# funkelab/cellulus

Measured on AMD Instinct MI355X. Metric: train crops/sec (U-Net fwd+bwd + OCE loss + Adam), higher is better.
Workload: dtype f32 (exact 3xbf16 operand split, 6 products, f32 accumulate)

## Files before the change

### cellulus_amd/_clx.py

```python

import ctypes
import os
from ctypes import POINTER, Structure, c_char_p, c_double, c_int, c_longlong, c_size_t, c_void_p

import torch

_HERE = os.path.dirname(os.path.abspath(__file__))
LIB_PATH = os.path.join(_HERE, "libclx.so")


class ClxError(RuntimeError):
    """A libclx entry point returned a negative status."""


class ClxSrc(Structure):

    _fields_ = [
        ("ptr", c_void_p),
        ("C", c_int),
        ("ld", c_int),
        ("D", c_int),
        ("H", c_int),
        ("W", c_int),
        ("oz", c_int),
        ("oy", c_int),
        ("ox", c_int),
        ("fz", c_int),
        ("fy", c_int),
        ("fx", c_int),
    ]


class ClxPackJob(Structure):

    _fields_ = [("w", c_void_p), ("wp", c_void_p), ("cout", c_int), ("cin", c_int), ("taps", c_int),
                ("cin_pad", c_int), ("cout_pad", c_int), ("mode", c_int)]


class ClxConvDesc(Structure):

    _fields_ = [
        ("nsrc", c_int),
        ("src", ClxSrc * 2),
        ("B", c_int),
        ("ID", c_int),
        ("IH", c_int),
        ("IW", c_int),
        ("KD", c_int),
        ("KH", c_int),
        ("KW", c_int),
        ("PD", c_int),
        ("PH", c_int),
        ("PW", c_int),
        ("N", c_int),
        ("wpack", c_void_p),
        ("bias", c_void_p),
        ("relu", c_int),
        ("mask", c_void_p),
        ("ld_mask", c_int),
        ("out", c_void_p),
        ("ld_out", c_int),
        ("accumulate", c_int),
        ("algo", c_int),
        ("workspace", c_void_p),
        ("workspace_bytes", c_size_t),
        ("vcache", c_void_p),
        ("vcache_valid", c_int),
        ("c_real", c_int),
        ("dy_vcache", c_void_p),
        ("gate_out", c_void_p),
        ("ld_gate", c_int),
        ("mask_bits", c_void_p),
        ("ld_mask_bits", c_int),
        ("det_turns", c_void_p),
        ("adjoint", c_int),
        ("pool_out", c_void_p),
        ("ld_pool", c_int),
        ("tile_list", c_void_p),
        ("tile_count", c_int),
        ("precision", c_int),
        ("wplanes", c_void_p),
        ("aplanes", c_void_p),
        ("aplanes_valid", c_int),
        ("dyplanes", c_void_p),
        ("dyplanes_valid", c_int),
        ("out_planes", c_void_p),
        ("out_colsum", c_void_p),
    ]


_P = c_void_p
_I = c_int
_LL = c_longlong
_D = c_double

PROTOTYPES = {
    "clx_last_error": (c_char_p, []),
    "clx_abi_version": (_I, []),
    "clx_device_count": (_I, []),
    "clx_profile_enable": (_I, [_I]),
    "clx_profile_read": (_I, [_I, POINTER(c_double), POINTER(c_double), POINTER(c_double)]),
    "clx_profile_clock": (_I, [POINTER(c_double), POINTER(c_double), _I]),
    "clx_conv_fwd": (_I, [POINTER(ClxConvDesc), _P]),
    "clx_conv_wgrad": (_I, [POINTER(ClxConvDesc), _P, _I, _P, _P, _P]),
    "clx_chain64_fwd": (_I, [_P, _I, _LL, _P, _P, _P, _I, _P, _I, _P, _P, _I, _I, _P, _I, _P, _I, _P]),
    "clx_chain64_bwd": (_I, [_P, _I, _I, _P, _I, _P, _I, _I, _LL, _P, _P, _P, _I, _P, _P, _P, _P, _P]),
    "clx_pack_weights": (_I, [_P, _P, _I, _I, _I, _I, _I, _I, _P]),
    "clx_pack_weights_batch": (_I, [_P, _I, _LL, _P]),
    "clx_unpack_wgrad": (_I, [_P, _P, _I, _I, _I, _I, _I, _P]),
    "clx_unpack_wgrad_wino": (_I, [_P, _P, _I, _I, _I, _I, _I, _I, _I, _P]),
    "clx_conv_workspace_bytes": (c_size_t, [POINTER(ClxConvDesc), _I]),
    "clx_conv_vcache_bytes": (c_size_t, [POINTER(ClxConvDesc), _I]),
    "clx_conv_sp_covers": (_I, [POINTER(ClxConvDesc), _I]),
    "clx_planes_bytes": (c_size_t, [_LL, _I]),
    "clx_split_planes": (_I, [_P, _LL, _LL, _I, _P, _P]),
    "clx_join_planes": (_I, [_P, _LL, _I, _P, _LL, _P]),
    "clx_gemm_planes": (_I, [_P, _P, _I, _I, _I, _P, _I, _P, _I, _P]),
    "clx_wgrad_planes": (_I, [_P, _P, _LL, _I, _I, _P, _I, _P]),
    "clx_conv_fused_applicable": (_I, [POINTER(ClxConvDesc)]),
    "clx_conv_fused_workspace_bytes": (c_size_t, [POINTER(ClxConvDesc)]),
    "clx_planar_to_pixel": (_I, [_P, _P, _I, _I, _LL, _I, _P]),
    "clx_pixel_to_planar": (_I, [_P, _P, _I, _I, _LL, _I, _P]),
    "clx_depth_to_space": (_I, [_P, _I, _P, _I, _I, _I, _I, _I, _I, _I, _I, _I, _P]),
    "clx_space_to_depth": (_I, [_P, _I, _P, _I, _I, _I, _I, _I, _I, _I, _I, _I, _P]),
    "clx_subpixel_split_weights": (_I, [_P, _P, _P] + [_I] * 10 + [_P]),
    "clx_subpixel_fold_grads": (_I, [_P, _P, _P] + [_I] * 10 + [_P]),
    "clx_maxpool_fwd": (_I, [_P, _P, _I, _I, _I, _I, _I, _I, _I, _I, _P]),
    "clx_changed_rows_workspace": (c_size_t, [_I, _I, _I, _I]),
    "clx_changed_rows": (_I, [_P, _P, _I, _I, _I, _I, _I, _I, _I, _I, _I, _P, _P, _LL, _P, _P]),
    "clx_changed_tiles": (_I, [_P, _I, _I, _I, _I, _I, _I, _I, _I, _I, _I, _I, _P, _P, _LL, _P]),
    "clx_grey_rows": (_I, [_P, _I, _I, _I, _I, _I, _P, _LL, _P, _P, _I, _I, _P, _I, _P]),
    "clx_conv_first_dgrad": (_I, [_P, _I, _P, _I, _I, _I, _I, _I, _I, _I, _P, _P]),
    "clx_gather_rows": (_I, [_P, _I, _P, _LL, _I, _P, _I, _P]),
    "clx_scatter_rows": (_I, [_P, _I, _P, _LL, _I, _P, _I, _P]),
    "clx_broadcast_rows": (_I, [_P, _LL, _P, _I, _P]),
    "clx_maxpool_bwd": (_I, [_P, _P, _P, _P] + [_I] * 7 + [_P] + [_I] * 8 + [_P]),
    "clx_upsample_bwd": (_I, [_P] + [_I] * 8 + [_P, _P] + [_I] * 8 + [_P]),
    "clx_gather_add_fwd": (_I, [_P, _P, _P, _I, _I, _I, _I, _I, _I, _P, _P]),
    "clx_gather_add_bwd": (_I, [_P, _P, _P, _I, _I, _I, _I, _I, _I, _P, _P]),
    "clx_oce_loss_fwd_bwd": (_I, [_P, _P, _P, _P, _LL, _I, ctypes.c_float, ctypes.c_float, ctypes.c_float, _P]),
    "clx_conv_wgrad_turns_bytes": (c_size_t, [POINTER(ClxConvDesc)]),
    "clx_colsum_scratch_bytes": (c_size_t, [_I]),
    "clx_colsum_ordered": (_I, [_P, _I, _LL, _I, _P, _P, _P]),
    "clx_oce_pairs_det_scratch_bytes": (c_size_t, [_I, _I, _LL]),
    "clx_oce_pairs_fused_det": (_I, [_P, _P, _P, _P, _P, _I, _I, _I, _I, _I, _I, ctypes.c_float, ctypes.c_float, _P, _P]),
    "clx_oce_pairs_fused": (_I, [_P, _P, _P, _P, _P, _I, _I, _I, _I, _I, _I, ctypes.c_float, ctypes.c_float, _P]),
    "clx_sample_pairs": (_I, [_P, _P, _P, _I, _I, _I, _I, _I, _I, POINTER(c_int), ctypes.c_ulonglong,
                              ctypes.c_ulonglong, _P]),
    "clx_adam_step": (_I, [_P, _P, _P, _P, _LL, _D, _D, _D, _D, _D, _I, _P]),
    "clx_adam_step_guarded": (_I, [_P, _P, _P, _P, _LL, _D, _D, _D, _D, _D, _I, _P, _P]),
    "clx_noise_stats": (_I, [_P, _P, _I, _I, _LL, _P]),
    "clx_noise_inject": (_I, [_P, _P, _P, _I, _I, _LL, ctypes.c_float, _P]),
    "clx_zero_many": (_I, [POINTER(_P), POINTER(_LL), _I, _P]),
    "clx_gather_rows_f64": (_I, [_P, _P, _LL, _I, _P, _P]),
    "clx_rows_extent_f64": (_I, [_P, _LL, _I, _P, _P]),
    "clx_noise_stats_minmax": (_I, [_P, _P, _I, _I, _LL, _P, _I, _P]),
    "clx_ms_prepare_workspace": (c_size_t, [_LL]),
    "clx_ms_prepare": (_I, [_P, _P, _D, _I, _I, _I, _I, _P, _P, _P, _P, _P]),
    "clx_ms_prepare_f32": (_I, [_P, _P, _D, _I, _I, _I, _I, _P, _P, _P, _P, _P]),
    "clx_ms_iterate": (_I, [_P, _I, _P, _I, _I, _D, _I, _P, _P, _P, _P]),
    "clx_ms_iterate_grid": (_I, [_P, _I, _P, POINTER(c_double), _D, _I, _I, _I, _P, _I, _I, _D, _I,
                                 _P, _P, _P, _P]),
    "clx_ms_assign": (_I, [_P, _P, _I, _P, _I, _I, _P, _P]),
    "clx_ms_assign_grid": (_I, [_P, _P, _I, _P, _I, _I, _P, _P, POINTER(c_double), _D, _I, _I, _I, _P, _P]),
    "clx_ms_assign_cells": (_I, [_P, _P, _I, _P, _I, _I, _P, _P, POINTER(c_double), _D, _I, _I, _I, _P, _P]),
    "clx_ms_assign_dense": (_I, [_P, _P, _I, _I, _P, _P, POINTER(c_double), _D, _I, _I, _I, _P, _I, _I, _I, _I, _P, _P]),
    "clx_ms_dedup_centers": (_I, [_P, _P, _I, _I, _D, _P, POINTER(_I)]),
    "clx_sample_offsets_mt19937": (_I, [_P, POINTER(_I), _I, _I, _LL, _P, POINTER(_I)]),
    "clx_elastic_crop_workspace": (c_size_t, [_I, POINTER(c_int), _I]),
    "clx_elastic_crop": (_I, [_P, _I, _I, _I, _I, POINTER(c_int), POINTER(c_int), POINTER(c_int), ctypes.c_float, _I, _I,
                              _P, _P, _P, _P, _P, _P]),
    "clx_ms_bucket_workspace": (c_size_t, [_I, _LL]),
    "clx_ms_bucket": (_I, [_P, _I, _I, POINTER(c_double), _D, _I, _I, _I, _P, _P, _P, _P]),
    "clx_offset_magnitude": (_I, [_P, _P, _I, _LL, _P]),
    "clx_gaussian_filter_f64": (_I, [_P, _P, _P, _I, _I, _I, _P, _I, _P]),
    "clx_negate_f64": (_I, [_P, _P, _LL, _P]),
    "clx_peak_local_max": (_I, [_P, _I, _I, _I, _P, _P, _I, _P, _P]),
    "clx_greedy_cluster": (_I, [_P, _P, _I, _I, _I, _D, _I, _D, _I, _P, _P, _P, _P]),
    "clx_cc_workspace": (c_size_t, [_LL]),
    "clx_cc_label_filter": (_I, [_P, _P, _I, _I, _I, _I, _P, _P, _P]),
    "clx_edt_workspace": (c_size_t, [_LL]),
    "clx_edt_sq": (_I, [_P, _P, _I, _I, _I, _I, _P, _P]),
    "clx_grow_shrink": (_I, [_P, _I, _I, _I, _I, _I, _P, _P]),
    "clx_minmax_f64": (_I, [_P, _LL, _P, _P]),
    "clx_histogram_f64": (_I, [_P, _LL, _P, _I, _P, _P]),
    "clx_minmax_f32": (_I, [_P, _LL, _P, _P]),
    "clx_histogram_f32": (_I, [_P, _LL, _P, _I, _P, _P]),
    "clx_inst_stats": (_I, [_P, _P, _I, _I, _I, _I, _I, _P, _P, _P]),
    "clx_inst_histogram": (_I, [_P, _P, _I, _LL, _P, _I, _P, _I, _P, _P]),
    "clx_inst_refine": (_I, [_P, _P, _I, _I, _I, _I, _I, _P, _P, _P, _P, _P, _I, _P, _P]),
    "clx_lz4_decompress": (_LL, [_P, _LL, _P, _LL]),
    "clx_blosclz_decompress": (_LL, [_P, _LL, _P, _LL]),
    "clx_blosc_compress_bound": (_LL, [_LL]),
    "clx_blosc_compress_lz4": (_LL, [_P, _LL, _I, _I, _P, _LL]),
    "clx_unshuffle_bytes": (_I, [_P, _P, _LL, _I]),
    "clx_label_presence": (_I, [_P, _LL, _I, _P, _P, _P]),
# ... 90 lines not shown
```

### cellulus_amd/csrc/clx_common.h

```cpp
#pragma once
#include <hip/hip_runtime.h>
#include <hip/hip_ext.h>
#include <stdint.h>
#include <stdio.h>
#include <stdarg.h>
#include "../../include/clx.h"

void clx_set_error(const char* fmt, ...);

#define CLX_REQUIRE(cond, ...)                \
  do {                                        \
    if (!(cond)) {                            \
      clx_set_error(__VA_ARGS__);             \
      return CLX_ERR_ARG;                     \
    }                                         \
  } while (0)

#define CLX_CHECK_LAUNCH(name)                                           \
  do {                                                                   \
    hipError_t e__ = hipGetLastError();                                  \
    if (e__ != hipSuccess) {                                             \
      clx_set_error("%s: launch failed: %s", name, hipGetErrorString(e__)); \
      return CLX_ERR_LAUNCH;                                             \
    }                                                                    \
  } while (0)

typedef float f32x4 __attribute__((ext_vector_type(4)));
typedef float f32x16 __attribute__((ext_vector_type(16)));

struct FastDiv {
  uint32_t m, l, d;
};
static inline FastDiv make_fastdiv(uint32_t d) {
  FastDiv f;
  f.d = d;
  uint32_t l = 0;
  while ((1ull << l) < d) ++l;
  f.l = l;
  f.m = (uint32_t)(((1ull << 32) * ((1ull << l) - d)) / d + 1);
  return f;
}
__device__ __forceinline__ uint32_t fdiv(uint32_t n, const FastDiv& f) {
  return (__umulhi(f.m, n) + n) >> f.l;
}

__device__ __forceinline__ int xcd_remap(int bid, int nblocks) {
  const int q = nblocks >> 3, r = nblocks & 7;
  const int xcd = bid & 7, idx = bid >> 3;
  const int base = (xcd < r) ? xcd * (q + 1) : r * (q + 1) + (xcd - r) * q;
  return base + idx;
}

static inline int cdiv(long long a, long long b) { return (int)((a + b - 1) / b); }

bool clx_smallc_applicable(const clx_conv_desc* d);
int clx_smallc_fwd(const clx_conv_desc* d, hipStream_t st);
int clx_smallc_wgrad(const clx_conv_desc* d, const float* dy, int ld_dy, float* dwpack,
                     float* dbias, hipStream_t st);

int clx_igemm_launch(const clx_conv_desc* d, int batch, long long bs_in, long long bs_w,
                     long long bs_out, hipStream_t st);
int clx_wgrad_launch(const clx_conv_desc* d, const float* dy, int ld_dy, float* dwpack, float* dbias,
                     int batch, long long bs_x, long long bs_dy, long long bs_out, hipStream_t st);
bool clx_sp_fwd_rule(const clx_conv_desc* d);
bool clx_sp_wgrad_rule(const clx_conv_desc* d);
bool clx_sp_applicable(const clx_conv_desc* d);
bool clx_wino_sp(const clx_conv_desc* d);
int clx_sp_launch(const void* A, const void* B, int M, int N, int K, long long rows_a, int batch, long long bs_a, long long bs_b,
                  long long bs_out, const clx_conv_desc* ep, hipStream_t st);
int clx_sp_clock_read(double* shader_ticks, double* wall_ticks, int reset);
int clx_sp_split(const float* x, long long ld, long long rows, int K, void* planes, float* colsum, int nreal, hipStream_t st);
int clx_sp_wgrad_launch(const void* dy_planes, const void* x_planes, long long rows, int N, int C, int batch, long long bs_dy,
                        long long bs_x, long long bs_out, float* dw, int ld_dw, hipStream_t st);
int clx_wino_fwd(const clx_conv_desc* d, hipStream_t st);
int clx_wino_wgrad(const clx_conv_desc* d, const float* dy, int ld_dy, float* dwpack, float* dbias,
                   hipStream_t st);
int clx_wino_pack(const float* w, float* wp, int cout, int cin, int cin_pad, int cout_pad, int dgrad, int tile,
                  int ksize, int kd, hipStream_t st);

int clx_wino_fused_fwd(const clx_conv_desc* d, hipStream_t st);

bool clx_prof_enabled();
void clx_prof_events(int kind, double flops, hipEvent_t* e0, hipEvent_t* e1);
#define CLX_LAUNCH_TIMED(kernel, grid, block, st, e0, e1, ...) \
  hipExtLaunchKernelGGL(kernel, grid, block, 0, st, e0, e1, 0, __VA_ARGS__)
#define CLX_LAUNCH_KIND(kind, kernel, grid, block, lds, st, ...)                              \
  do {                                                                                        \
    hipEvent_t e0__ = nullptr, e1__ = nullptr;                                                \
    if (clx_prof_enabled()) clx_prof_events(kind, 0.0, &e0__, &e1__);                         \
    hipExtLaunchKernelGGL(kernel, grid, block, lds, st, e0__, e1__, 0, __VA_ARGS__);          \
  } while (0)
```

### cellulus_amd/csrc/conv_igemm.hip

```cpp
#include "clx_common.h"
#include <stdlib.h>

__device__ unsigned long long g_clk_ticks[2];
extern "C" int clx_profile_clock(double* shader_ticks, double* wall_ticks_100mhz, int reset) {
  unsigned long long h[2] = {0ull, 0ull};
  if (hipMemcpyFromSymbol(h, HIP_SYMBOL(g_clk_ticks), sizeof(h)) != hipSuccess) {
    clx_set_error("clx_profile_clock: copy failed");
    return CLX_ERR_LAUNCH;
  }
  double sc = 0.0, sw = 0.0;
  if (clx_sp_clock_read(&sc, &sw, reset) != CLX_OK) {
    clx_set_error("clx_profile_clock: copy failed");
    return CLX_ERR_LAUNCH;
  }
  if (shader_ticks) *shader_ticks = (double)h[0] + sc;
  if (wall_ticks_100mhz) *wall_ticks_100mhz = (double)h[1] + sw;
  if (reset) {
    const unsigned long long z[2] = {0ull, 0ull};
    if (hipMemcpyToSymbol(HIP_SYMBOL(g_clk_ticks), z, sizeof(z)) != hipSuccess) {
      clx_set_error("clx_profile_clock: reset failed");
      return CLX_ERR_LAUNCH;
    }
  }
  return CLX_OK;
// ... 400 lines not shown
    } else if (n_live) {
#pragma unroll 1
      for (int j = 0; j < PH; ++j) {
        if (!live[j]) continue;
        float* dst = out_base + (size_t)mrow[j] * p.ld_out;
        for (int e = 0; e < 4 && n + e < p.N; ++e) {
          float x = val[j][e];
          if (p.mask) x = (p.mask[(size_t)mrow[j] * p.ld_mask + n + e] > 0.f) ? x : 0.f;
          dst[e] = x;
        }
      }
    }
  }
  if (clk_block) { atomicAdd(&g_clk_ticks[0], clock64() - clk_c0); atomicAdd(&g_clk_ticks[1], wall_clock64() - clk_w0); }
}

}

static const float* zero_buffer() {
  static const float* cache[64] = {nullptr};
  int dev = 0;
  if (hipGetDevice(&dev) != hipSuccess || dev < 0 || dev >= 64) return nullptr;
  if (cache[dev] == nullptr) {
    void* ptr = nullptr;
    if (hipGetSymbolAddress(&ptr, HIP_SYMBOL(g_zero16)) != hipSuccess) return nullptr;
    cache[dev] = (const float*)ptr;
  }
  return cache[dev];
}

static int conv_validate(const clx_conv_desc* d, const char* who) {
  CLX_REQUIRE(d != nullptr, "%s: null descriptor", who);
  CLX_REQUIRE(d->nsrc == 1 || d->nsrc == 2, "%s: nsrc must be 1 or 2", who);
  CLX_REQUIRE(d->B > 0 && d->ID > 0 && d->IH > 0 && d->IW > 0, "%s: bad extent", who);
  const int K[3] = {d->KD, d->KH, d->KW};
  const int P[3] = {d->PD, d->PH, d->PW};
  const int I[3] = {d->ID, d->IH, d->IW};
  for (int i = 0; i < 3; ++i) {
    CLX_REQUIRE(K[i] >= 1 && K[i] <= 3, "%s: kernel extent must be 1, 2 or 3", who);
    CLX_REQUIRE(P[i] >= 0 && P[i] < K[i], "%s: padding must be < kernel extent", who);
    CLX_REQUIRE(I[i] + 2 * P[i] - K[i] + 1 > 0, "%s: input smaller than kernel", who);
  }
  for (int s = 0; s < d->nsrc; ++s) {
    const clx_src& S = d->src[s];
    CLX_REQUIRE(S.ptr != nullptr, "%s: null source %d", who, s);
    CLX_REQUIRE(S.C > 0 && S.C % 4 == 0 && S.ld % 4 == 0 && S.ld >= S.C,
                "%s: source channels/ld must be multiples of 4 (C=%d ld=%d)", who, S.C, S.ld);
    CLX_REQUIRE(((uintptr_t)S.ptr & 15) == 0, "%s: source pointer must be 16-byte aligned", who);
    CLX_REQUIRE(S.fz >= 1 && S.fy >= 1 && S.fx >= 1, "%s: upsample factors >= 1", who);
    CLX_REQUIRE(S.oz >= 0 && S.oy >= 0 && S.ox >= 0, "%s: negative crop", who);
    CLX_REQUIRE((d->ID - 1 + S.oz) / S.fz < S.D && (d->IH - 1 + S.oy) / S.fy < S.H &&
                    (d->IW - 1 + S.ox) / S.fx < S.W,
                "%s: source %d smaller than the logical input", who, s);
  }
  const long long M = (long long)d->B * (d->ID + 2 * d->PD - d->KD + 1) *
                      (d->IH + 2 * d->PH - d->KH + 1) * (d->IW + 2 * d->PW - d->KW + 1);
  CLX_REQUIRE(M < (1ll << 31), "%s: too many output pixels", who);
  return CLX_OK;
}

static void fill_params(const clx_conv_desc* d, ConvP& p) {
  p.nsrc = d->nsrc;
  for (int s = 0; s < 2; ++s) {
    const clx_src& S = d->src[s < d->nsrc ? s : 0];
    p.src[s] = SrcP{S.ptr, S.C, S.ld, S.D, S.H, S.W, S.oz, S.oy, S.ox, S.fz, S.fy, S.fx};
  }
  p.B = d->B; p.ID = d->ID; p.IH = d->IH; p.IW = d->IW;
  p.KD = d->KD; p.KH = d->KH; p.KW = d->KW;
  p.PD = d->PD; p.PH = d->PH; p.PW = d->PW;
  p.OD = d->ID + 2 * d->PD - d->KD + 1;
  p.OH = d->IH + 2 * d->PH - d->KH + 1;
  p.OW = d->IW + 2 * d->PW - d->KW + 1;
  p.N = d->N;
  p.M = d->B * p.OD * p.OH * p.OW;
  p.Ctot = d->src[0].C + (d->nsrc == 2 ? d->src[1].C : 0);
  p.Ktot = p.Ctot * d->KD * d->KH * d->KW;
  p.dOW = make_fastdiv(p.OW); p.dOH = make_fastdiv(p.OH); p.dOD = make_fastdiv(p.OD);
  p.wpack = d->wpack; p.bias = d->bias; p.mask = d->mask; p.out = d->out;
  p.gate_out = d->gate_out; p.ld_gate = d->ld_gate; p.mask_bits = d->mask_bits; p.ld_mask_bits = d->ld_mask_bits;
  p.relu = d->relu; p.ld_mask = d->ld_mask; p.ld_out = d->ld_out;
  p.accumulate = d->accumulate;
  p.bs_in = p.bs_w = p.bs_out = 0;
  p.flush_every = 0;
}

extern "C" int clx_conv_fwd(const clx_conv_desc* d, clx_stream stream) {
  int rc = conv_validate(d, "clx_conv_fwd");
  if (rc) return rc;
  CLX_REQUIRE(d->wpack && d->out, "clx_conv_fwd: null wpack/out");
  CLX_REQUIRE(d->N > 0 && d->ld_out >= d->N, "clx_conv_fwd: bad N/ld_out");
  CLX_REQUIRE(((uintptr_t)d->wpack & 15) == 0, "clx_conv_fwd: wpack must be 16-byte aligned");
  CLX_REQUIRE(d->mask == nullptr || (d->ld_mask >= d->N && d->ld_mask % 4 == 0 &&
                                     ((uintptr_t)d->mask & 15) == 0),
              "clx_conv_fwd: mask must be 16-byte aligned with ld_mask %% 4 == 0 and >= N");
  CLX_REQUIRE(d->ld_out % 4 == 0 && ((uintptr_t)d->out & 15) == 0,
              "clx_conv_fwd: out must be 16-byte aligned with ld_out %% 4 == 0");
  CLX_REQUIRE(d->gate_out == nullptr || (d->relu && d->ld_out % 32 == 0 && d->ld_gate * 32 >= d->ld_out),
              "clx_conv_fwd: gate_out needs relu, ld_out %% 32 == 0 and ld_gate >= ld_out / 32");
  CLX_REQUIRE(d->mask_bits == nullptr || (d->mask == nullptr && d->ld_mask_bits * 32 >= d->N),
              "clx_conv_fwd: mask_bits replaces mask and needs ld_mask_bits >= ceil(N / 32)");
  CLX_REQUIRE(d->algo == CLX_ALGO_DIRECT || d->algo == CLX_ALGO_WINOGRAD || d->algo == CLX_ALGO_WINOGRAD4 ||
                  d->algo == CLX_ALGO_WINOGRAD4_FUSED,
              "clx_conv_fwd: bad algo");
  CLX_REQUIRE((d->out_planes == nullptr && d->out_colsum == nullptr && !d->aplanes_valid) ||
                  (d->algo == CLX_ALGO_DIRECT && d->aplanes != nullptr && clx_sp_applicable(d)),
              "clx_conv_fwd: out_planes / out_colsum / aplanes_valid need the split-precision 1x1 product "
              "(clx_conv_sp_covers, wplanes and aplanes)");
  if (d->algo == CLX_ALGO_WINOGRAD4_FUSED) return clx_wino_fused_fwd(d, (hipStream_t)stream);
  if (d->algo != CLX_ALGO_DIRECT) return clx_wino_fwd(d, (hipStream_t)stream);
  CLX_REQUIRE(d->pool_out == nullptr && d->tile_list == nullptr && !d->adjoint,
              "clx_conv_fwd: pool_out / tile_list / adjoint need a Winograd algorithm (algo = %d)", d->algo);
  if (clx_smallc_applicable(d) && d->mask == nullptr && d->mask_bits == nullptr && d->gate_out == nullptr) {
    clx_smallc_fwd(d, (hipStream_t)stream);
    CLX_CHECK_LAUNCH("clx_conv_fwd(small-channel)");
    return CLX_OK;
  }
  rc = clx_igemm_launch(d, 1, 0, 0, 0, (hipStream_t)stream);
  if (rc) return rc;
  CLX_CHECK_LAUNCH("clx_conv_fwd");
  return CLX_OK;
}

int clx_igemm_launch(const clx_conv_desc* d, int batch, long long bs_in, long long bs_w,
                     long long bs_out, hipStream_t st) {
  if (batch == 1 && d->aplanes != nullptr && clx_sp_applicable(d)) {
    const clx_src& S = d->src[0];
    const long long M = (long long)d->B * d->ID * d->IH * d->IW;
    if (!d->aplanes_valid) {
      const int rc = clx_sp_split(S.ptr, S.ld, M, S.C, d->aplanes, nullptr, 0, st);
      if (rc) return rc;
    }
    return clx_sp_launch(d->aplanes, d->wplanes, (int)M, d->N, S.C, M, 1, 0, 0, 0, d, st);
  }
  ConvP p;
  fill_params(d, p);
  p.zeros = zero_buffer();
  CLX_REQUIRE(p.zeros != nullptr, "clx_conv_fwd: cannot resolve the device zero buffer");
  p.bs_in = bs_in; p.bs_w = bs_w; p.bs_out = bs_out;
  static const int flush_env = getenv("CLX_IGEMM_FLUSH") ? atoi(getenv("CLX_IGEMM_FLUSH")) : 2;
  p.flush_every = flush_env > 0 ? flush_env : 0;
  const bool wide = d->N > 64 && (double)(cdiv(d->N, 128) * 128) / d->N <= 1.2;
  hipEvent_t e0 = nullptr, e1 = nullptr;
  if (clx_prof_enabled())
    clx_prof_events(wide ? CLX_PROF_IGEMM_WIDE : CLX_PROF_IGEMM_NARROW, 2.0 * p.M * p.N * p.Ktot * batch, &e0, &e1);
  static const bool fast_env = getenv("CLX_IGEMM_FAST") == nullptr || atoi(getenv("CLX_IGEMM_FAST")) != 0;
  int fast = fast_env && (long long)p.N * p.Ktot < (1ll << 30) ? 1 : 0;
  const bool padded = d->PD != 0 || d->PH != 0 || d->PW != 0;
  for (int s = 0; s < d->nsrc && fast; ++s) {
    const clx_src& S = d->src[s];
    const long long floats = (long long)d->B * S.D * S.H * S.W * S.ld;
    if (S.C % BK != 0 || floats >= (padded ? (1ll << 29) : (1ll << 30))) fast = 0;
  }
  if (fast && padded) fast = 2;
  static const bool dbg = getenv("CLX_IGEMM_DEBUG") != nullptr;
  if (dbg) fprintf(stderr, "igemm fast=%d wide=%d M=%d N=%d K=%d batch=%d pad=%d%d%d k=%d%d%d nsrc=%d C0=%d\n", (int)fast, (int)wide, p.M, p.N, p.Ktot, batch, d->PD, d->PH, d->PW, d->KD, d->KH, d->KW, d->nsrc, d->src[0].C);
  if (wide) {
    p.nbm = cdiv(p.M, 128); p.nbn = cdiv(p.N, 128);
    if (fast == 1) CLX_LAUNCH_TIMED((conv_igemm_kernel<128, 128, 2, 2, 1>), dim3(p.nbm * p.nbn, batch), dim3(256), st, e0, e1, p);
    else if (fast == 2) CLX_LAUNCH_TIMED((conv_igemm_kernel<128, 128, 2, 2, 2>), dim3(p.nbm * p.nbn, batch), dim3(256), st, e0, e1, p);
    else CLX_LAUNCH_TIMED((conv_igemm_kernel<128, 128, 2, 2>), dim3(p.nbm * p.nbn, batch), dim3(256), st, e0, e1, p);
  } else {
    p.nbm = cdiv(p.M, 128); p.nbn = cdiv(p.N, 64);
    if (fast == 1) CLX_LAUNCH_TIMED((conv_igemm_kernel<128, 64, 4, 1, 1>), dim3(p.nbm * p.nbn, batch), dim3(256), st, e0, e1, p);
    else if (fast == 2) CLX_LAUNCH_TIMED((conv_igemm_kernel<128, 64, 4, 1, 2>), dim3(p.nbm * p.nbn, batch), dim3(256), st, e0, e1, p);
    else CLX_LAUNCH_TIMED((conv_igemm_kernel<128, 64, 4, 1>), dim3(p.nbm * p.nbn, batch), dim3(256), st, e0, e1, p);
  }
  return CLX_OK;
}
```

### cellulus_amd/csrc/conv_smallc.hip

```cpp
#include "clx_common.h"

namespace {

struct SmallP {
  const float* x;
  int ld_x, B, D, H, W;
  int oz, oy, ox;
  int ID, IH, IW, KD, KH, KW, PD, PH, PW, OD, OH, OW;
  int N, M, taps;
  FastDiv dOW, dOH, dOD;
  const float* wpack;
  const float* bias;
  float* out;
  int ld_out, relu;
  const float* dy;
  int ld_dy;
  float* dwp;
  float* dbias;
  int tiles_per_block;
  int RX, items;
  FastDiv dRX;
};

constexpr int PT = 64;
constexpr int MAX_TAPS = 27;

template <int PTILE>
__device__ __forceinline__ void stage_patch(const SmallP& p, int m0, float* Xs) {
  static_assert(256 % PTILE == 0, "a thread keeps one pixel of the tile");
  const int K4 = p.taps;
  const int pl = threadIdx.x % PTILE;
  const uint32_t m = (uint32_t)(m0 + pl);
  const bool live = m < (uint32_t)p.M;
  const uint32_t q1 = fdiv(m, p.dOW);
  const int ox = (int)(m - q1 * p.OW);
  const uint32_t q2 = fdiv(q1, p.dOH);
  const int oy = (int)(q1 - q2 * p.OH);
  const uint32_t q3 = fdiv(q2, p.dOD);
  const int oz = (int)(q2 - q3 * p.OD);
  const int b = (int)q3;
  int tx = 0, ty = 0, tz = 0;
  {
    const int tap = threadIdx.x / PTILE;
    tx = tap % p.KW; ty = (tap / p.KW) % p.KH; tz = tap / (p.KW * p.KH);
  }
  constexpr int STEP = 256 / PTILE;
  for (int tap = threadIdx.x / PTILE; tap < K4; tap += STEP) {
    f32x4 v = {0.f, 0.f, 0.f, 0.f};
    const int lz = oz + tz - p.PD, ly = oy + ty - p.PH, lx = ox + tx - p.PW;
    if (live && (unsigned)lz < (unsigned)p.ID && (unsigned)ly < (unsigned)p.IH && (unsigned)lx < (unsigned)p.IW) {
      const long long pix = (((long long)b * p.D + lz + p.oz) * p.H + ly + p.oy) * p.W + lx + p.ox;
      v = *reinterpret_cast<const f32x4*>(p.x + pix * p.ld_x);
    }
    *reinterpret_cast<f32x4*>(&Xs[(pl * K4 + tap) * 4]) = v;
    tx += STEP;
    while (tx >= p.KW) { tx -= p.KW; if (++ty == p.KH) { ty = 0; ++tz; } }
  }
}

template <int NG>
__global__ __launch_bounds__(256) void conv_smallc_fwd_kernel(const SmallP p) {
  constexpr int PL = 256 / NG;
  constexpr int PPT = PT / PL;
  extern __shared__ float smem[];
  const int K = p.taps * 4;
  float* Ws = smem;
  float* Xs = smem + K * NG * 4;
  const int n0 = blockIdx.y * NG * 4;
  const int ng = threadIdx.x % NG, pl = threadIdx.x / NG;
  __shared__ int used_channels;
  if (threadIdx.x == 0) used_channels = 0;
  __syncthreads();
  int mine_used = 0;
  for (int idx = threadIdx.x; idx < K * NG * 4; idx += 256) {
    const int n = idx / K, k = idx % K;
    const float wv = (n0 + n < p.N) ? p.wpack[(size_t)(n0 + n) * K + k] : 0.f;
    Ws[k * NG * 4 + n] = wv;
    if (wv != 0.f) mine_used |= 1 << (k & 3);
  }
  if (mine_used) atomicOr(&used_channels, mine_used);
  const int n = n0 + ng * 4;
  f32x4 bv = {0.f, 0.f, 0.f, 0.f};
  if (p.bias && n < p.N) {
#pragma unroll
    for (int e = 0; e < 4; ++e) bv[e] = (n + e < p.N) ? p.bias[n + e] : 0.f;
  }
  for (int t = 0; t < p.tiles_per_block; ++t) {
    const int m0 = (blockIdx.x * p.tiles_per_block + t) * PT;
    if (m0 >= p.M) break;
    __syncthreads();
    stage_patch<PT>(p, m0, Xs);
    __syncthreads();
    f32x4 acc[PPT];
#pragma unroll
    for (int i = 0; i < PPT; ++i) acc[i] = bv;
    const int used = used_channels;
    for (int c = 0; c < 4; ++c) {
// ... 47 lines not shown
  const long long per = (long long)p.tiles_per_block;
  const long long m_begin = (long long)blockIdx.x * per;
  const long long m_end = m_begin + per < p.M ? m_begin + per : p.M;
  const bool live = n < p.N;
  const int gtap = tap0 + (g < ntap ? g : 0);
  const int my_tx = gtap % p.KW - p.PW, my_ty = (gtap / p.KW) % p.KH - p.PH, my_tz = gtap / (p.KW * p.KH) - p.PD;
  for (long long mm = m_begin + q; mm < m_end; mm += Q) {
    const uint32_t m = (uint32_t)mm;
    const uint32_t q1 = fdiv(m, p.dOW);
    const int ox = (int)(m - q1 * p.OW);
    const uint32_t q2 = fdiv(q1, p.dOH);
    const int oy = (int)(q1 - q2 * p.OH);
    const uint32_t q3 = fdiv(q2, p.dOD);
    const int oz = (int)(q2 - q3 * p.OD);
    const int b = (int)q3;
    f32x4 dyv = {0.f, 0.f, 0.f, 0.f};
    if (live) dyv = *reinterpret_cast<const f32x4*>(p.dy + (size_t)m * p.ld_dy + n);
    if (tap0 == 0) bsum += dyv;
    if constexpr (G >= 16) {
      f32x4 mine = {0.f, 0.f, 0.f, 0.f};
      if (g < ntap) {
        const int lz = oz + my_tz, ly = oy + my_ty, lx = ox + my_tx;
        if ((unsigned)lz < (unsigned)p.ID && (unsigned)ly < (unsigned)p.IH && (unsigned)lx < (unsigned)p.IW) {
          const long long pix = (((long long)b * p.D + lz + p.oz) * p.H + ly + p.oy) * p.W + lx + p.ox;
          mine = *reinterpret_cast<const f32x4*>(p.x + pix * p.ld_x);
        }
      }
#pragma unroll
      for (int a = 0; a < MT; ++a) {
        if (a < ntap) {
          f32x4 xv;
#pragma unroll
          for (int c = 0; c < 4; ++c) {
            xv[c] = __shfl(mine[c], (int)(threadIdx.x & 63 & ~(G - 1)) + a, 64);
          }
#pragma unroll
          for (int c = 0; c < 4; ++c) acc[a][c] += xv[c] * dyv;
        }
      }
    } else {
#pragma unroll
      for (int a = 0; a < MT; ++a) {
        if (a < ntap) {
          const int tap = tap0 + a;
          const int lz = oz + tap / (p.KW * p.KH) - p.PD, ly = oy + (tap / p.KW) % p.KH - p.PH, lx = ox + tap % p.KW - p.PW;
          f32x4 xv = {0.f, 0.f, 0.f, 0.f};
          if ((unsigned)lz < (unsigned)p.ID && (unsigned)ly < (unsigned)p.IH && (unsigned)lx < (unsigned)p.IW) {
            const long long pix = (((long long)b * p.D + lz + p.oz) * p.H + ly + p.oy) * p.W + lx + p.ox;
            xv = *reinterpret_cast<const f32x4*>(p.x + pix * p.ld_x);
          }
#pragma unroll
          for (int c = 0; c < 4; ++c) acc[a][c] += xv[c] * dyv;
        }
      }
    }
  }
  __syncthreads();
#pragma unroll
  for (int a = 0; a < MT; ++a) {
    if (a < ntap) {
#pragma unroll
      for (int c = 0; c < 4; ++c)
#pragma unroll
        for (int e = 0; e < 4; ++e) atomicAdd(&red[(a * 4 + c) * NT + g * 4 + e], acc[a][c][e]);
    }
  }
#pragma unroll
  for (int e = 0; e < 4; ++e) atomicAdd(&red[ntap * 4 * NT + g * 4 + e], bsum[e]);
  __syncthreads();
  for (int i = threadIdx.x; i < ntap * 4 * NT; i += 256) {
    const int nl = i % NT, c = (i / NT) & 3, tap = tap0 + i / (4 * NT);
    if (n0 + nl < p.N) atomicAdd(p.dwp + ((size_t)tap * p.N + n0 + nl) * 4 + c, red[i]);
  }
  if (p.dbias && tap0 == 0)
    for (int i = threadIdx.x; i < NT; i += 256)
      if (n0 + i < p.N) atomicAdd(p.dbias + n0 + i, red[ntap * 4 * NT + i]);
}

struct Run {
  int ox0, m0;
  long long base;
};

__device__ __forceinline__ Run decode_run(const SmallP& p, uint32_t item) {
  const uint32_t q1 = fdiv(item, p.dRX);
  const int rx = (int)(item - q1 * p.RX);
  const uint32_t q2 = fdiv(q1, p.dOH);
  const int oy = (int)(q1 - q2 * p.OH);
  const uint32_t q3 = fdiv(q2, p.dOD);
  const int oz = (int)(q2 - q3 * p.OD);
  const int b = (int)q3;
  Run r;
  r.ox0 = rx * 4;
  r.m0 = ((b * p.OD + oz) * p.OH + oy) * p.OW + r.ox0;
  r.base = (((long long)b * p.D + oz + p.oz) * p.H + oy + p.oy) * p.W + r.ox0 + p.ox;
  return r;
}

template <int KD>
struct GreyLane {
  static constexpr int R = KD * 3, NP = R * 6, TAPS = R * 3;
  int px, cq, col;
  long long poff;
  __device__ __forceinline__ GreyLane(const SmallP& p) {
    const int lane = threadIdx.x & 63;
    px = lane >> 4; cq = lane & 15;
    const int l = lane < NP ? lane : 0;
    const int r = l / 6;
    col = l - r * 6;
    const int tz = r / 3, ty = r - tz * 3;
    poff = ((long long)tz * p.H + ty) * p.W;
  }
  __device__ __forceinline__ float load_patch(const SmallP& p, const Run& r) const {
    const int c = r.ox0 + col < p.IW ? col : p.IW - 1 - r.ox0;
    return p.x[(r.base + poff + c) * p.ld_x];
  }
  __device__ __forceinline__ float tap(float pv, int row, int tx) const {
    return __shfl(pv, row * 6 + tx + px, 64);
  }
};

template <int KD>
__global__ __launch_bounds__(256) void conv_grey_fwd_kernel(const SmallP p) {
  using L = GreyLane<KD>;
  const L ln(p);
  const int wave = __builtin_amdgcn_readfirstlane(threadIdx.x >> 6);
  const int n = blockIdx.y * 64 + ln.cq * 4;
  const bool live_n = n < p.N;
  f32x4 w[L::TAPS];
#pragma unroll
  for (int t = 0; t < L::TAPS; ++t)
#pragma unroll
    for (int e = 0; e < 4; ++e) w[t][e] = live_n ? p.wpack[((size_t)(n + e) * L::TAPS + t) * 4] : 0.f;
  f32x4 bv = {0.f, 0.f, 0.f, 0.f};
  if (p.bias && live_n) bv = *reinterpret_cast<const f32x4*>(p.bias + n);
  const uint32_t last = (uint32_t)p.items - 1, stride = gridDim.x * 4;
  uint32_t item = blockIdx.x * 4 + wave;
  Run r[3];
  float pv[3];
#pragma unroll
  for (int s = 0; s < 2; ++s) {
    r[s] = decode_run(p, item + s * stride < last ? item + s * stride : last);
    pv[s] = ln.load_patch(p, r[s]);
  }
  while (true) {
#pragma unroll
    for (int s = 0; s < 3; ++s) {
      if (item > last) return;
      const int s2 = (s + 2) % 3;
      const uint32_t nxt = item + 2 * stride;
      r[s2] = decode_run(p, nxt < last ? nxt : last);
      pv[s2] = ln.load_patch(p, r[s2]);
      f32x4 acc = bv;
#pragma unroll
      for (int row = 0; row < L::R; ++row)
#pragma unroll
        for (int tx = 0; tx < 3; ++tx) acc += ln.tap(pv[s], row, tx) * w[row * 3 + tx];
      if (p.relu) {
#pragma unroll
        for (int e = 0; e < 4; ++e) acc[e] = fmaxf(acc[e], 0.f);
      }
      if (live_n && r[s].ox0 + ln.px < p.OW)
        *reinterpret_cast<f32x4*>(p.out + (size_t)(r[s].m0 + ln.px) * p.ld_out + n) = acc;
      item += stride;
    }
  }
}

template <int KD>
__global__ __launch_bounds__(256) void conv_grey_wgrad_kernel(const SmallP p) {
  using L = GreyLane<KD>;
  __shared__ float red[(L::TAPS + 1) * 64];
  const L ln(p);
  const int wave = __builtin_amdgcn_readfirstlane(threadIdx.x >> 6);
  const int n0 = blockIdx.y * 64, n = n0 + ln.cq * 4;
  const bool live_n = n < p.N;
  const int nld = live_n ? n : 0;
  for (int i = threadIdx.x; i < (L::TAPS + 1) * 64; i += 256) red[i] = 0.f;
  f32x4 acc[L::TAPS];
#pragma unroll
  for (int t = 0; t < L::TAPS; ++t) acc[t] = f32x4{0.f, 0.f, 0.f, 0.f};
  f32x4 bsum = {0.f, 0.f, 0.f, 0.f};
  const uint32_t last = (uint32_t)p.items - 1, stride = gridDim.x * 4;
  uint32_t item = blockIdx.x * 4 + wave;
  auto load_dy = [&](const Run& r) {
    const int m = r.ox0 + ln.px < p.OW ? r.m0 + ln.px : r.m0;
    return *reinterpret_cast<const f32x4*>(p.dy + (size_t)m * p.ld_dy + nld);
  };
  Run r[3];
  float pv[3];
  f32x4 dy[3];
#pragma unroll
  for (int s = 0; s < 2; ++s) {
    r[s] = decode_run(p, item + s * stride < last ? item + s * stride : last);
    pv[s] = ln.load_patch(p, r[s]);
    dy[s] = load_dy(r[s]);
  }
  bool more = item <= last;
  while (more) {
#pragma unroll
    for (int s = 0; s < 3; ++s) {
      if (more) {
        const int s2 = (s + 2) % 3;
        const uint32_t nxt = item + 2 * stride;
        r[s2] = decode_run(p, nxt < last ? nxt : last);
        pv[s2] = ln.load_patch(p, r[s2]);
        dy[s2] = load_dy(r[s2]);
        const bool ok = live_n && r[s].ox0 + ln.px < p.OW;
        f32x4 dyv;
#pragma unroll
        for (int e = 0; e < 4; ++e) dyv[e] = ok ? dy[s][e] : 0.f;
        bsum += dyv;
#pragma unroll
        for (int row = 0; row < L::R; ++row)
#pragma unroll
          for (int tx = 0; tx < 3; ++tx) acc[row * 3 + tx] += ln.tap(pv[s], row, tx) * dyv;
        item += stride;
        more = item <= last;
      }
    }
  }
  __syncthreads();
#pragma unroll
  for (int t = 0; t < L::TAPS; ++t)
#pragma unroll
    for (int e = 0; e < 4; ++e) atomicAdd(&red[t * 64 + ln.cq * 4 + e], acc[t][e]);
#pragma unroll
  for (int e = 0; e < 4; ++e) atomicAdd(&red[L::TAPS * 64 + ln.cq * 4 + e], bsum[e]);
  __syncthreads();
  for (int i = threadIdx.x; i < L::TAPS * 64; i += 256) {
    const int nl = i & 63, t = i >> 6;
    if (n0 + nl < p.N) atomicAdd(p.dwp + ((size_t)t * p.N + n0 + nl) * 4, red[i]);
  }
  if (p.dbias && threadIdx.x < 64 && n0 + threadIdx.x < p.N)
    atomicAdd(p.dbias + n0 + threadIdx.x, red[L::TAPS * 64 + threadIdx.x]);
}

template <int KD>
__global__ __launch_bounds__(256) void conv_grey_rows_kernel(const float* __restrict__ x, int D, int H, int W, int OD,
                                                             int OH, int OW, const int* __restrict__ rows, long long n,
                                                             const float* __restrict__ wpack,
                                                             const float* __restrict__ bias, int relu, int N,
                                                             float* __restrict__ out, int ld_out) {
  constexpr int R = KD * 3, TAPS = R * 3;
  const int lane = threadIdx.x & 63, px = lane >> 4, cq = lane & 15;
  const int nn = blockIdx.y * 64 + cq * 4;
  const bool live_n = nn < N;
  f32x4 w[TAPS];
#pragma unroll
  for (int t = 0; t < TAPS; ++t)
#pragma unroll
    for (int e = 0; e < 4; ++e) w[t][e] = live_n ? wpack[((size_t)(nn + e) * TAPS + t) * 4] : 0.f;
  f32x4 bv = {0.f, 0.f, 0.f, 0.f};
  if (bias && live_n) bv = *reinterpret_cast<const f32x4*>(bias + nn);
  const long long npo = (long long)OD * OH * OW;
  const long long groups = (n + 3) / 4;
  for (long long g = (long long)blockIdx.x * 4 + (threadIdx.x >> 6); g < groups; g += (long long)gridDim.x * 4) {
    const long long r = g * 4 + px;
    const bool live = r < n;
    const long long row = rows[live ? r : n - 1];
    const long long b = row / npo, pix = row - b * npo;
    const int ox = (int)(pix % OW), oy = (int)((pix / OW) % OH), oz = (int)(pix / ((long long)OW * OH));
    const float* src = x + ((b * D + oz) * H + oy) * (long long)W + ox;
    float xv[TAPS];
#pragma unroll
    for (int rr = 0; rr < R; ++rr)
#pragma unroll
      for (int tx = 0; tx < 3; ++tx) xv[rr * 3 + tx] = src[((long long)(rr / 3) * H + (rr % 3)) * W + tx];
    f32x4 acc = bv;
#pragma unroll
    for (int rr = 0; rr < R; ++rr)
#pragma unroll
      for (int tx = 0; tx < 3; ++tx) acc += xv[rr * 3 + tx] * w[rr * 3 + tx];
    if (relu) {
#pragma unroll
      for (int e = 0; e < 4; ++e) acc[e] = fmaxf(acc[e], 0.f);
    }
    if (live && live_n) *reinterpret_cast<f32x4*>(out + (size_t)r * ld_out + nn) = acc;
  }
}

bool grey_applicable(const clx_conv_desc* d, int ld_act) {
  return d->c_real == 1 && d->KH == 3 && d->KW == 3 && (d->KD == 1 || d->KD == 3) && d->PD == 0 &&
         d->PH == 0 && d->PW == 0 && d->N % 4 == 0 && ld_act % 4 == 0;
}

dim3 grey_grid(SmallP& p) {
  p.RX = cdiv(p.OW, 4);
  p.items = p.B * p.OD * p.OH * p.RX;
  p.dRX = make_fastdiv(p.RX);
  const int ny = cdiv(p.N, 64);
  int nx = 768 / ny;
  if (nx < 1) nx = 1;
  if (nx > cdiv(p.items, 4)) nx = cdiv(p.items, 4);
  return dim3(nx, ny);
}

bool fill(const clx_conv_desc* d, SmallP& p) {
  const clx_src& S = d->src[0];
  p.x = S.ptr; p.ld_x = S.ld; p.B = d->B; p.D = S.D; p.H = S.H; p.W = S.W;
  p.oz = S.oz; p.oy = S.oy; p.ox = S.ox;
  p.ID = d->ID; p.IH = d->IH; p.IW = d->IW;
  p.KD = d->KD; p.KH = d->KH; p.KW = d->KW;
  p.PD = d->PD; p.PH = d->PH; p.PW = d->PW;
  p.OD = d->ID + 2 * d->PD - d->KD + 1;
  p.OH = d->IH + 2 * d->PH - d->KH + 1;
  p.OW = d->IW + 2 * d->PW - d->KW + 1;
  p.N = d->N;
  p.M = d->B * p.OD * p.OH * p.OW;
  p.taps = d->KD * d->KH * d->KW;
  p.dOW = make_fastdiv(p.OW); p.dOH = make_fastdiv(p.OH); p.dOD = make_fastdiv(p.OD);
  return true;
}

int pick_ng(int N) {
  int ng = 4;
  while (ng < 64 && ng * 4 < N) ng *= 2;
  return ng;
}

}

bool clx_smallc_applicable(const clx_conv_desc* d) {
  if (d->nsrc != 1 || d->accumulate) return false;
  const clx_src& S = d->src[0];
  if (S.C != 4 || S.fz != 1 || S.fy != 1 || S.fx != 1) return false;
  const int taps = d->KD * d->KH * d->KW;
  return taps > 1 && taps <= MAX_TAPS && d->N >= 4;
}

int clx_smallc_fwd(const clx_conv_desc* d, hipStream_t st) {
  SmallP p{};
  fill(d, p);
  p.wpack = d->wpack; p.bias = d->bias; p.out = d->out; p.ld_out = d->ld_out; p.relu = d->relu;
  if (grey_applicable(d, d->ld_out) && ((uintptr_t)d->out & 15) == 0 && (!d->bias || ((uintptr_t)d->bias & 15) == 0)) {
    const dim3 grid = grey_grid(p);
    if (d->KD == 1) conv_grey_fwd_kernel<1><<<grid, 256, 0, st>>>(p);
    else conv_grey_fwd_kernel<3><<<grid, 256, 0, st>>>(p);
    return CLX_OK;
  }
  const int ng = pick_ng(p.N);
  const int K = p.taps * 4;
  const int tiles = cdiv(p.M, PT);
  p.tiles_per_block = tiles > 4096 ? 4 : 1;
  const dim3 grid(cdiv(tiles, p.tiles_per_block), cdiv(p.N, ng * 4));
  const size_t lds = (size_t)(K * ng * 4 + PT * K) * sizeof(float);
  switch (ng) {
    case 4: conv_smallc_fwd_kernel<4><<<grid, 256, lds, st>>>(p); break;
    case 8: conv_smallc_fwd_kernel<8><<<grid, 256, lds, st>>>(p); break;
    case 16: conv_smallc_fwd_kernel<16><<<grid, 256, lds, st>>>(p); break;
    case 32: conv_smallc_fwd_kernel<32><<<grid, 256, lds, st>>>(p); break;
    default: conv_smallc_fwd_kernel<64><<<grid, 256, lds, st>>>(p); break;
  }
  return CLX_OK;
}

int clx_smallc_wgrad(const clx_conv_desc* d, const float* dy, int ld_dy, float* dwpack,
                     float* dbias, hipStream_t st) {
  SmallP p{};
  fill(d, p);
  p.dy = dy; p.ld_dy = ld_dy; p.dwp = dwpack; p.dbias = dbias;
  if (grey_applicable(d, ld_dy) && ((uintptr_t)dy & 15) == 0) {
    const dim3 grid = grey_grid(p);
    if (d->KD == 1) conv_grey_wgrad_kernel<1><<<grid, 256, 0, st>>>(p);
    else conv_grey_wgrad_kernel<3><<<grid, 256, 0, st>>>(p);
    return CLX_OK;
  }
  const int ng = pick_ng(p.N);
  const int blocks = p.M < 512 * 64 ? cdiv(p.M, 64) : 512;
  p.tiles_per_block = cdiv(p.M, blocks);
  const dim3 grid(cdiv(p.M, p.tiles_per_block), cdiv(p.N, ng * 4), cdiv(p.taps, 9));
  const size_t lds = (size_t)((p.taps < 9 ? p.taps : 9) * 4 * ng * 4 + ng * 4) * sizeof(float);
  switch (ng) {
    case 4: conv_smallc_wgrad_stream_kernel<4><<<grid, 256, lds, st>>>(p); break;
    case 8: conv_smallc_wgrad_stream_kernel<8><<<grid, 256, lds, st>>>(p); break;
    case 16: conv_smallc_wgrad_stream_kernel<16><<<grid, 256, lds, st>>>(p); break;
    case 32: conv_smallc_wgrad_stream_kernel<32><<<grid, 256, lds, st>>>(p); break;
    default: conv_smallc_wgrad_stream_kernel<64><<<grid, 256, lds, st>>>(p); break;
  }
  return CLX_OK;
}

extern "C" int clx_grey_rows(const float* x, int B, int ID, int IH, int IW, int KD, const int* rows, long long n,
                             const float* wpack, const float* bias, int relu, int N, float* out, int ld_out,
                             clx_stream stream) {
  CLX_REQUIRE(n >= 0, "clx_grey_rows: bad count");
  if (n == 0) return CLX_OK;
  CLX_REQUIRE(x && rows && wpack && out, "clx_grey_rows: null pointer");
  CLX_REQUIRE(B > 0 && (KD == 1 || KD == 3) && ID >= KD && IH >= 3 && IW >= 3, "clx_grey_rows: a 3x3 or 3x3x3 window");
  CLX_REQUIRE(N > 0 && N % 4 == 0 && ld_out % 4 == 0 && ld_out >= N && ((uintptr_t)out & 15) == 0 &&
                  (!bias || ((uintptr_t)bias & 15) == 0),
              "clx_grey_rows: N, ld_out multiples of 4, aligned out / bias");
  const int OD = ID - KD + 1, OH = IH - 2, OW = IW - 2;
  long long gx = (n + 15) / 16;
  if (gx > 4096) gx = 4096;
  const dim3 grid((unsigned)gx, (unsigned)((N + 63) / 64));
  hipStream_t st = (hipStream_t)stream;
  if (KD == 1) conv_grey_rows_kernel<1><<<grid, 256, 0, st>>>(x, ID, IH, IW, OD, OH, OW, rows, n, wpack, bias, relu, N, out, ld_out);
  else conv_grey_rows_kernel<3><<<grid, 256, 0, st>>>(x, ID, IH, IW, OD, OH, OW, rows, n, wpack, bias, relu, N, out, ld_out);
  CLX_CHECK_LAUNCH("clx_grey_rows");
  return CLX_OK;
}
```

### cellulus_amd/csrc/gemm_sp.hip

```cpp
#include "clx_common.h"
#include "sp_planes.h"
#include <stdlib.h>
#include <type_traits>

__device__ unsigned long long g_sp_clk_ticks[2];
int clx_sp_clock_read(double* shader_ticks, double* wall_ticks, int reset) {
  unsigned long long h[2] = {0ull, 0ull};
  if (hipMemcpyFromSymbol(h, HIP_SYMBOL(g_sp_clk_ticks), sizeof(h)) != hipSuccess) return CLX_ERR_LAUNCH;
  *shader_ticks = (double)h[0];
  *wall_ticks = (double)h[1];
  if (reset) {
    const unsigned long long z[2] = {0ull, 0ull};
    if (hipMemcpyToSymbol(HIP_SYMBOL(g_sp_clk_ticks), z, sizeof(z)) != hipSuccess) return CLX_ERR_LAUNCH;
  }
  return CLX_OK;
}

namespace {

typedef __bf16 bf16x8 __attribute__((ext_vector_type(8)));
using sp::u32x2;
using sp::u32x4;
using sp::FRAG;
using sp::KSTEP;
// ... 31 lines not shown
    if constexpr (COLSUM) { s0 += v0; s1 += v1; }
    u32x2 a0, a1, a2, b0, b1, b2;
    split4(v0, a0, a1, a2);
    split4(v1, b0, b1, b2);
    char* dst = out + f * KSTEP + lane * 16;
    *reinterpret_cast<u32x4*>(dst) = u32x4{a0[0], a0[1], b0[0], b0[1]};
    *reinterpret_cast<u32x4*>(dst + FRAG) = u32x4{a1[0], a1[1], b1[0], b1[1]};
    *reinterpret_cast<u32x4*>(dst + 2 * FRAG) = u32x4{a2[0], a2[1], b2[0], b2[1]};
  }
  if constexpr (COLSUM) {
    if (w0 < nfrag) {
      const int ks = (int)(w0 % ksteps);
#pragma unroll
      for (int e = 0; e < 4; ++e) {
#pragma unroll
        for (int m = 1; m < 32; m <<= 1) { s0[e] += __shfl_xor(s0[e], m, 64); s1[e] += __shfl_xor(s1[e], m, 64); }
      }
      if (r == 0) {
#pragma unroll
        for (int e = 0; e < 4; ++e) {
          const int k0 = ks * 16 + h * 8 + e;
          if (k0 < nreal) atomicAdd(colsum + k0, s0[e]);
          if (k0 + 4 < nreal) atomicAdd(colsum + k0 + 4, s1[e]);
        }
      }
    }
  }
}

__global__ __launch_bounds__(256) void sp_join_kernel(const char* __restrict__ in, long long ld, long long rows, int ksteps,
                                                      float* __restrict__ x, long long nfrag) {
  const int lane = threadIdx.x & 63;
  const long long w0 = ((long long)blockIdx.x * blockDim.x + threadIdx.x) >> 6, nw = ((long long)gridDim.x * blockDim.x) >> 6;
  const int r = lane & 31, h = lane >> 5;
  for (long long f = w0; f < nfrag; f += nw) {
    const int ks = (int)(f % ksteps);
    const long long rb = f / ksteps;
    const long long row = rb * 32 + r;
    if (row >= rows) continue;
    const char* src = in + f * KSTEP + lane * 16;
    const u32x4 q0 = *reinterpret_cast<const u32x4*>(src), q1 = *reinterpret_cast<const u32x4*>(src + FRAG),
                q2 = *reinterpret_cast<const u32x4*>(src + 2 * FRAG);
    float* dst = x + row * ld + ks * 16 + h * 8;
#pragma unroll
    for (int e = 0; e < 8; ++e) {
      const int sh = (e & 1) * 16;
      const float f0 = __uint_as_float(((q0[e >> 1] >> sh) & 0xffffu) << 16);
      const float f1 = __uint_as_float(((q1[e >> 1] >> sh) & 0xffffu) << 16);
      const float f2 = __uint_as_float(((q2[e >> 1] >> sh) & 0xffffu) << 16);
      dst[e] = (f0 + f1) + f2;
    }
  }
}

__global__ __launch_bounds__(256) void sp_zero_tail_kernel(char* __restrict__ planes, long long bs, long long rows, int ksteps) {
  const long long rb0 = rows >> 5, rb1 = sp::padded_rows(rows) / 32;
  const int per_rb = ksteps * 6 * 32;
  const long long total = (rb1 - rb0) * per_rb;
  for (long long i = (long long)blockIdx.x * blockDim.x + threadIdx.x; i < total; i += (long long)gridDim.x * blockDim.x) {
    const long long rb = rb0 + i / per_rb;
    const int k = (int)(i % per_rb), r = k & 31, q = k >> 5;
    if (rb * 32 + r >= rows)
      *reinterpret_cast<u32x4*>(planes + blockIdx.y * bs + rb * ksteps * (long long)KSTEP + (long long)q * 512 + r * 16) = u32x4{0u, 0u, 0u, 0u};
  }
}

struct SpP {
  const char* A;
  const char* B;
  long long bs_a, bs_b, bs_out;
  float* out;
  int M, N, ksteps;
  int rb_a;
  int rb_b;
  const float* bias;
  const float* mask;
  const unsigned int* mask_bits;
  unsigned int* gate_out;
  const float* zeros;
  int relu, accumulate, ld_out, ld_mask, ld_mask_bits, ld_gate;
  int nbm, nbn;
  char* out_planes;
  float* colsum; int colsum_n;
  unsigned int stride_a, stride_b;
  int total_steps, steps_per_slice, nslices;
};

template <int BM = SP_BM, int NWAVES = 8, int BN = SP_BN>
__device__ __forceinline__ void sp_epilogue_from_lds(const SpP& p, const float* Cs, int m0, int n0, int batch, int tid, int lane) {
  constexpr int WPR = BN / 32;
  constexpr int LDC = BN + 4;
  constexpr int PASS_ROWS = NWAVES / WPR * 8;
  constexpr int ITERS = BM / PASS_ROWS;
  constexpr int PH = 8;
  static_assert(ITERS % PH == 0, "whole groups of passes");
  const int wv = tid >> 6;
  const int c4 = (wv % WPR) * 32 + (lane & 7) * 4;
  const int row0 = (wv / WPR) * 8 + (lane >> 3);
  const int n = n0 + c4;
  const bool n_live = n < p.N;
  f32x4 csum = {0.f, 0.f, 0.f, 0.f};
  const long long prow = p.out_planes ? sp::padded_rows(p.M) : 0;
#pragma unroll 1
  for (int h0 = 0; h0 < ITERS; h0 += PH) {
    f32x4 val[PH];
    int mrow[PH];
    bool live[PH];
#pragma unroll
    for (int j = 0; j < PH; ++j) {
      const int row = row0 + PASS_ROWS * (h0 + j);
      mrow[j] = m0 + row;
      live[j] = mrow[j] < p.M && n_live;
      val[j] = *reinterpret_cast<const f32x4*>(&Cs[row * LDC + c4]);
    }
    float* const out_base = p.out + batch * p.bs_out + n;
    if (p.accumulate) {
      f32x4 prev[PH];
#pragma unroll
      for (int j = 0; j < PH; ++j)
        prev[j] = *reinterpret_cast<const f32x4*>(live[j] ? out_base + (size_t)mrow[j] * p.ld_out : p.zeros);
#pragma unroll
      for (int j = 0; j < PH; ++j) val[j] += prev[j];
    }
    if (p.relu) {
#pragma unroll
      for (int j = 0; j < PH; ++j)
#pragma unroll
        for (int e = 0; e < 4; ++e) val[j][e] = fmaxf(val[j][e], 0.f);
    }
    if (p.mask_bits) {
      unsigned int wd[PH];
#pragma unroll
      for (int j = 0; j < PH; ++j) wd[j] = live[j] ? p.mask_bits[(size_t)mrow[j] * p.ld_mask_bits + (n >> 5)] : 0u;
#pragma unroll
      for (int j = 0; j < PH; ++j)
#pragma unroll
        for (int e = 0; e < 4; ++e) val[j][e] = ((wd[j] >> ((n & 31) + e)) & 1u) ? val[j][e] : 0.f;
    }
    if (p.gate_out) {
#pragma unroll
      for (int j = 0; j < PH; ++j) {
        unsigned int nib = 0u;
#pragma unroll
        for (int e = 0; e < 4; ++e) nib |= (live[j] && val[j][e] > 0.f) ? (1u << e) : 0u;
        unsigned int word = nib << (4 * (lane & 7));
        word |= __shfl_xor(word, 1, 64);
        word |= __shfl_xor(word, 2, 64);
        word |= __shfl_xor(word, 4, 64);
        if ((lane & 7) == 0 && mrow[j] < p.M && n_live) p.gate_out[(size_t)mrow[j] * p.ld_gate + (n >> 5)] = word;
      }
    }
    if (p.mask) {
      f32x4 mk[PH];
#pragma unroll
      for (int j = 0; j < PH; ++j)
        mk[j] = *reinterpret_cast<const f32x4*>(live[j] ? p.mask + (size_t)mrow[j] * p.ld_mask + n : p.zeros);
#pragma unroll
      for (int j = 0; j < PH; ++j)
#pragma unroll
        for (int e = 0; e < 4; ++e) val[j][e] = (!live[j] || mk[j][e] > 0.f) ? val[j][e] : 0.f;
    }
#pragma unroll
    for (int j = 0; j < PH; ++j)
      if (live[j]) *reinterpret_cast<f32x4*>(out_base + (size_t)mrow[j] * p.ld_out) = val[j];
    if (p.out_planes) {
#pragma unroll
      for (int j = 0; j < PH; ++j)
        if (n_live && mrow[j] < prow)
          sp::store4(p.out_planes, mrow[j], n, p.N >> 4, live[j] ? val[j] : f32x4{0.f, 0.f, 0.f, 0.f});
    }
    if (p.colsum) {
#pragma unroll
      for (int j = 0; j < PH; ++j)
        if (live[j]) csum += val[j];
    }
  }
  if (p.colsum) {
#pragma unroll
    for (int e = 0; e < 4; ++e) {
      csum[e] += __shfl_xor(csum[e], 8, 64);
      csum[e] += __shfl_xor(csum[e], 16, 64);
      csum[e] += __shfl_xor(csum[e], 32, 64);
    }
    if ((lane >> 3) == 0 && n_live) {
#pragma unroll
      for (int e = 0; e < 4; ++e)
        if (n + e < p.colsum_n) atomicAdd(p.colsum + n + e, csum[e]);
    }
  }
}

template <int MODE>
__global__ __launch_bounds__(512, 1) void gemm_sp_kernel(const SpP p) {
  __shared__ __attribute__((aligned(16))) char smem[RING * STAGE];
  const int tid = threadIdx.x, lane = tid & 63;
  const int w = __builtin_amdgcn_readfirstlane(tid >> 6);
  const int wm = w >> 1, wn = w & 1;
  int tile_m, tile_n, batch, step0 = 0, ksteps;
  if constexpr (MODE == 0) {
    const int v = xcd_remap(blockIdx.x, p.nbm * p.nbn);
    tile_n = v % p.nbn; tile_m = v / p.nbn;
    batch = blockIdx.y;
    ksteps = p.ksteps;
  } else {
    const int T = p.nbm * p.nbn;
    const int u = xcd_remap(blockIdx.x, gridDim.x);
    const int per_batch = T * p.nslices;
    batch = u / per_batch;
    const int v = u % per_batch;
    const int slice = v / T, t = v % T;
    tile_n = t % p.nbn; tile_m = t / p.nbn;
    step0 = slice * p.steps_per_slice;
    ksteps = p.total_steps - step0 < p.steps_per_slice ? p.total_steps - step0 : p.steps_per_slice;
  }
  const int m0 = tile_m * SP_BM, n0 = tile_n * SP_BN;
  const bool clk_block = blockIdx.x == gridDim.x / 2 && blockIdx.y == gridDim.y / 2 && threadIdx.x == 0;
  unsigned long long clk_c0 = 0, clk_w0 = 0;
  if (clk_block) { clk_c0 = clock64(); clk_w0 = wall_clock64(); }

  const char* const Ab = p.A + batch * p.bs_a;
  const char* const Bb = p.B + batch * p.bs_b;
  auto frag_base = [&](int f) __attribute__((always_inline)) -> const char* {
    if constexpr (MODE == 0) {
      if (f < A_FRAGS) {
        int rb = tile_m * (SP_BM / 32) + f / 3;
        if (rb > p.rb_a - 1) rb = p.rb_a - 1;
        return Ab + ((long long)rb * ksteps * 3 + f % 3) * FRAG;
      }
      const int g = f - A_FRAGS;
      int nb = tile_n * (SP_BN / 32) + g / 3;
      if (nb > p.rb_b - 1) nb = p.rb_b - 1;
      return Bb + ((long long)nb * ksteps * 3 + g % 3) * FRAG;
    } else {
      if (f < A_FRAGS) {
        int cb = tile_m * (SP_BM / 32) + f / 3;
        if (cb > p.M / 32 - 1) cb = p.M / 32 - 1;
        return Ab + ((long long)(2 * cb) * 3 + f % 3) * FRAG;
      }
      const int g = f - A_FRAGS;
      int cb = tile_n * (SP_BN / 32) + g / 3;
      if (cb > p.N / 32 - 1) cb = p.N / 32 - 1;
      return Bb + ((long long)(2 * cb) * 3 + g % 3) * FRAG;
    }
  };
  const char* gsrc[5];
#pragma unroll
  for (int q = 0; q < 4; ++q) gsrc[q] = frag_base(w + 8 * q);
// ... 704 lines not shown
  long long blocks = (nfrag + 3) / 4;
  if (blocks > 8192) blocks = 8192;
  if (colsum != nullptr) {
    if (blocks > 2048) blocks = 2048;
    int g = ksteps % 4 == 0 ? 4 : ksteps % 2 == 0 ? 2 : 1;
    const long long unit = ksteps / g;
    blocks = (blocks + unit - 1) / unit * unit;
    CLX_LAUNCH_KIND(CLX_PROF_SPLIT_PLANES, sp_split_kernel<true>, dim3((unsigned)blocks), dim3(256), 0, st, x, ld, rows, ksteps, (char*)planes,
                    nfrag, colsum, nreal);
  } else {
    CLX_LAUNCH_KIND(CLX_PROF_SPLIT_PLANES, sp_split_kernel<false>, dim3((unsigned)blocks), dim3(256), 0, st, x, ld, rows, ksteps, (char*)planes,
                    nfrag, (float*)nullptr, 0);
  }
  return CLX_OK;
}

extern "C" int clx_split_planes(const float* x, long long ld, long long rows, int K, void* planes, clx_stream stream) {
  const int rc = clx_sp_split(x, ld, rows, K, planes, nullptr, 0, (hipStream_t)stream);
  if (rc) return rc;
  CLX_CHECK_LAUNCH("clx_split_planes");
  return CLX_OK;
}

extern "C" int clx_join_planes(const void* planes, long long rows, int K, float* x, long long ld, clx_stream stream) {
  CLX_REQUIRE(x != nullptr && planes != nullptr, "clx_join_planes: null pointer");
  CLX_REQUIRE(rows > 0 && K > 0 && K % 16 == 0 && ld >= K, "clx_join_planes: K must be a multiple of 16, ld >= K");
  const long long nfrag = sp::padded_rows(rows) / 32 * (K / 16);
  long long blocks = (nfrag + 3) / 4;
  if (blocks > 8192) blocks = 8192;
  sp_join_kernel<<<dim3((unsigned)blocks), dim3(256), 0, (hipStream_t)stream>>>((const char*)planes, ld, rows, K / 16, x, nfrag);
  CLX_CHECK_LAUNCH("clx_join_planes");
  return CLX_OK;
}

static bool sp_pointwise(const clx_conv_desc* d) {
  if ((d->precision != CLX_PREC_F32X3BF16 && d->precision != CLX_PREC_F32X3BF16_G64) || d->nsrc != 1) return false;
  if (d->KD != 1 || d->KH != 1 || d->KW != 1 || d->PD || d->PH || d->PW) return false;
  const clx_src& S = d->src[0];
  if (S.fz != 1 || S.fy != 1 || S.fx != 1 || S.oz || S.oy || S.ox) return false;
  return S.D == d->ID && S.H == d->IH && S.W == d->IW;
}

bool clx_sp_fwd_rule(const clx_conv_desc* d) {
  if (!sp_pointwise(d)) return false;
  const bool g64 = d->precision == CLX_PREC_F32X3BF16_G64;
  return d->N % (g64 ? 64 : SP_BN) == 0 && d->N >= 128 && d->src[0].C % 64 == 0 && d->src[0].C >= 128 && d->ld_out % 4 == 0;
}

bool clx_sp_wgrad_rule(const clx_conv_desc* d) {
  if (!sp_pointwise(d)) return false;
  const int granule = d->precision == CLX_PREC_F32X3BF16_G64 ? 64 : 128;
  if (d->N % granule != 0 || d->src[0].C % granule != 0 || d->N < 128 || d->src[0].C < 128) return false;
  const long long ch = d->N > d->src[0].C ? d->N : d->src[0].C;
  return (long long)d->B * d->ID * d->IH * d->IW * ch * 6 < (1ll << 32) - (1 << 24);
}

bool clx_sp_applicable(const clx_conv_desc* d) { return d->wplanes != nullptr && clx_sp_fwd_rule(d); }

extern "C" int clx_conv_sp_covers(const clx_conv_desc* d, int pass) {
  if (d == nullptr || (pass != CLX_PASS_FWD && pass != CLX_PASS_WGRAD)) return 0;
  if (d->algo == CLX_ALGO_WINOGRAD || d->algo == CLX_ALGO_WINOGRAD4) return clx_wino_sp(d) ? 1 : 0;
  if (d->algo != CLX_ALGO_DIRECT) return 0;
  return (pass == CLX_PASS_FWD ? clx_sp_fwd_rule(d) : clx_sp_wgrad_rule(d)) ? 1 : 0;
}

int clx_sp_launch(const void* A, const void* B, int M, int N, int K, long long rows_a, int batch, long long bs_a, long long bs_b,
                  long long bs_out, const clx_conv_desc* ep, hipStream_t st) {
  CLX_REQUIRE(M > 0 && N > 0 && N % 64 == 0 && K >= 128 && K % 64 == 0,
              "clx_gemm_planes: needs N %% 64 == 0 (whole 128-wide tiles: N %% 128 == 0), K %% 64 == 0 and K >= 128");
  CLX_REQUIRE(rows_a >= M, "clx_gemm_planes: the A planes hold fewer rows than M");
  SpP p = {};
  p.A = (const char*)A; p.B = (const char*)B;
  p.bs_a = bs_a; p.bs_b = bs_b; p.bs_out = bs_out;
  p.out = ep->out; p.ld_out = ep->ld_out;
  p.M = M; p.N = N; p.ksteps = K / 16;
  p.rb_a = (int)(sp::padded_rows(rows_a) / 32);
  p.rb_b = (int)(sp::padded_rows(N) / 32);
  p.bias = ep->bias; p.mask = ep->mask; p.mask_bits = ep->mask_bits; p.gate_out = ep->gate_out;
  p.relu = ep->relu; p.accumulate = ep->accumulate; p.ld_mask = ep->ld_mask; p.ld_mask_bits = ep->ld_mask_bits; p.ld_gate = ep->ld_gate;
  p.zeros = sp_zero_buffer();
  CLX_REQUIRE(p.zeros != nullptr, "clx_gemm_planes: cannot resolve the device zero buffer");
  p.out_planes = batch == 1 ? (char*)ep->out_planes : nullptr;
  p.colsum = batch == 1 ? ep->out_colsum : nullptr; p.colsum_n = N;
  CLX_REQUIRE(p.out_planes == nullptr || ep->ld_out == N, "clx_gemm_planes: out_planes needs a dense output (ld_out == N)");
  p.nbm = cdiv(M, SP_BM); p.nbn = cdiv(N, SP_BN);
  const char* const tile_env = getenv("CLX_SP_TILE");
  const int tile_choice = tile_env != nullptr ? atoi(tile_env) : 0;
  const char* const maxk_env = getenv("CLX_SP_TILE_MAXK");
  const int maxk = maxk_env != nullptr ? atoi(maxk_env) : 1024;
  const bool small_tiles = tile_choice == 128 || (tile_choice != 256 && K <= maxk);
  const char* const shape_env = getenv("CLX_SP_MFMA");
  const bool mfma16 = shape_env != nullptr && atoi(shape_env) == 16 && N % SP_BN == 0;
  hipEvent_t e0 = nullptr, e1 = nullptr;
  if (clx_prof_enabled())
    clx_prof_events(small_tiles && !mfma16 ? CLX_PROF_GEMM_SP2 : CLX_PROF_GEMM_SP, 2.0 * M * N * K * batch, &e0, &e1);
  if (mfma16) CLX_LAUNCH_TIMED(gemm_sp16_kernel, dim3(p.nbm * p.nbn, batch), dim3(512), st, e0, e1, p);
  else if (small_tiles && N % 128 == 0) CLX_LAUNCH_TIMED(gemm_sp2_kernel<128>, dim3(cdiv(M, S2_BM) * (N / 128), batch), dim3(256), st, e0, e1, p);
  else if (small_tiles) CLX_LAUNCH_TIMED(gemm_sp2_kernel<64>, dim3(cdiv(M, S2_BM) * (N / 64), batch), dim3(256), st, e0, e1, p);
  else CLX_LAUNCH_TIMED(gemm_sp_kernel<0>, dim3(p.nbm * p.nbn, batch), dim3(512), st, e0, e1, p);
  return CLX_OK;
}

int clx_sp_wgrad_launch(const void* dy_planes, const void* x_planes, long long rows, int N, int C, int batch, long long bs_dy,
                        long long bs_x, long long bs_out, float* dw, int ld_dw, hipStream_t st) {
  CLX_REQUIRE(rows > 0 && N > 0 && C >= 128 && N % 64 == 0 && C % 64 == 0,
              "clx_wgrad_planes: needs N %% 64 == 0, C %% 64 == 0 and C >= 128");
  SpP p = {};
  p.A = (const char*)dy_planes; p.B = (const char*)x_planes;
  p.bs_a = bs_dy; p.bs_b = bs_x; p.bs_out = bs_out;
  p.out = dw; p.ld_out = ld_dw;
  p.M = N; p.N = C;
  p.stride_a = (unsigned int)(N / 16) * KSTEP; p.stride_b = (unsigned int)(C / 16) * KSTEP;
  CLX_REQUIRE(sp::planes_bytes(rows, N) < (1ll << 32) && sp::planes_bytes(rows, C) < (1ll << 32), "clx_wgrad_planes: operand planes beyond 4 GB");
  p.total_steps = (int)(sp::padded_rows(rows) / 16);
  p.nbm = cdiv(N, SP_BM); p.nbn = cdiv(C, SP_BN);
  const int tiles = p.nbm * p.nbn * batch;
  int cus = 256, dev = 0;
  if (hipGetDevice(&dev) == hipSuccess) (void)hipDeviceGetAttribute(&cus, hipDeviceAttributeMultiprocessorCount, dev);
  int best_ns = 1;
  double best = 1e30;
  const int max_ns = p.total_steps / 8 > 0 ? p.total_steps / 8 : 1;
  for (int ns = 1; ns <= max_ns && ns <= 4096; ++ns) {
    const int sps = (cdiv(p.total_steps, ns) + 7) / 8 * 8;
    const int real_ns = cdiv(p.total_steps, sps);
    if (p.total_steps - (real_ns - 1) * sps < 8) continue;
    const double cost = (double)cdiv((long long)tiles * real_ns, cus) * (sps + 12);
    if (cost < best) { best = cost; best_ns = ns; }
    if ((long long)tiles * ns > 16ll * cus) break;
  }
  p.steps_per_slice = (cdiv(p.total_steps, best_ns) + 7) / 8 * 8;
  p.nslices = cdiv(p.total_steps, p.steps_per_slice);
  CLX_REQUIRE(p.total_steps >= 8 && p.total_steps - (p.nslices - 1) * p.steps_per_slice >= 8, "clx_wgrad_planes: internal: a slice of fewer than 8 steps");
  hipEvent_t e0 = nullptr, e1 = nullptr;
  if (clx_prof_enabled()) clx_prof_events(CLX_PROF_WGRAD_SP, 2.0 * rows * N * C * batch, &e0, &e1);
  CLX_LAUNCH_TIMED(gemm_sp_kernel<1>, dim3(p.nbm * p.nbn * p.nslices * batch), dim3(512), st, e0, e1, p);
  return CLX_OK;
}

extern "C" int clx_wgrad_planes(const void* dy_planes, const void* x_planes, long long rows, int N, int C, float* dw, int ld_dw,
                                clx_stream stream) {
  CLX_REQUIRE(dy_planes && x_planes && dw && ld_dw >= C, "clx_wgrad_planes: null pointer / ld_dw < C");
  const int rc = clx_sp_wgrad_launch(dy_planes, x_planes, rows, N, C, 1, 0, 0, 0, dw, ld_dw, (hipStream_t)stream);
  if (rc) return rc;
  CLX_CHECK_LAUNCH("clx_wgrad_planes");
  return CLX_OK;
}

extern "C" int clx_gemm_planes(const void* a_planes, const void* b_planes, int M, int N, int K, const float* bias, int relu,
                               float* out, int ld_out, clx_stream stream) {
  CLX_REQUIRE(a_planes && b_planes && out, "clx_gemm_planes: null pointer");
  CLX_REQUIRE(ld_out >= N && ld_out % 4 == 0 && ((uintptr_t)out & 15) == 0, "clx_gemm_planes: out must be 16-byte aligned, ld_out %% 4 == 0");
  clx_conv_desc ep = {};
  ep.out = out; ep.ld_out = ld_out; ep.bias = bias; ep.relu = relu;
  const int rc = clx_sp_launch(a_planes, b_planes, M, N, K, M, 1, 0, 0, 0, &ep, (hipStream_t)stream);
  if (rc) return rc;
  CLX_CHECK_LAUNCH("clx_gemm_planes");
  return CLX_OK;
}
```

### cellulus_amd/csrc/wino.hip

```cpp
#include "clx_common.h"
#include "sp_planes.h"
#include "wino_tables.h"

namespace {

inline int grid_for(long long total, int block) {
  long long g = (total + block - 1) / block;
  if (g > 16384) g = 16384;
  if (g < 1) g = 1;
  return (int)g;
}

__device__ __forceinline__ f32x4 ld4(const float* p) { return *reinterpret_cast<const f32x4*>(p); }
__device__ __forceinline__ void st4(float* p, f32x4 v) { *reinterpret_cast<f32x4*>(p) = v; }

struct Geom {
  int B, SH, SW, oy, ox;
  int ID, SD, oz;
  int IH, IW, P;
  int OH, OW, th, tw;
  long long T;
};

template <int MT, int R, bool PL = false>
__global__ __launch_bounds__(256) void wino_input_kernel(const float* __restrict__ x, int ld_x, int C4, Geom g,
                                                         float* __restrict__ V, long long total,
                                                         const int* __restrict__ tile_list = nullptr, long long Tc = 0,
                                                         long long plane_bytes = 0) {
  using W = WT<MT, R>;
  constexpr int A = W::A;
  const int C = C4 * 4;
  const long long Trows = tile_list ? Tc : g.T;
  const long long plane = Trows * C;
  for (long long i = (long long)blockIdx.x * blockDim.x + threadIdx.x; i < total;
       i += (long long)gridDim.x * blockDim.x) {
    int c;
    long long t;
    if constexpr (PL) {
      sp::item_to_row_channel(i, C, t, c);
      if (t >= Trows) continue;
    } else {
      c = (int)(i % C4) * 4;
      t = i / C4;
    }
    const long long tg = tile_list ? (long long)tile_list[t] : t;
    const int tx = (int)(tg % g.tw);
    const long long q = tg / g.tw;
    const int ty = (int)(q % g.th);
    const int b = (int)(q / g.th);
    const int bb = b / g.ID, bz = b - bb * g.ID;
    f32x4 d[A][A];
#pragma unroll
    for (int r = 0; r < A; ++r) {
      const int ly = MT * ty - g.P + r;
#pragma unroll
      for (int s = 0; s < A; ++s) {
        const int lx = MT * tx - g.P + s;
        f32x4 v = {0.f, 0.f, 0.f, 0.f};
        if ((unsigned)ly < (unsigned)g.IH && (unsigned)lx < (unsigned)g.IW) {
          const long long pix = (((long long)bb * g.SD + bz + g.oz) * g.SH + ly + g.oy) * g.SW + lx + g.ox;
          v = ld4(x + pix * ld_x + c);
        }
        d[r][s] = v;
      }
    }
    f32x4 w[A][A];
#pragma unroll
    for (int s = 0; s < A; ++s)
#pragma unroll
      for (int r = 0; r < A; ++r) {
        f32x4 acc = {0.f, 0.f, 0.f, 0.f};
        bool first = true;
#pragma unroll
        for (int k = 0; k < A; ++k) axpy(acc, first, W::BT[r][k], d[k][s]);
        w[r][s] = acc;
      }
    float* dst = V + t * C + c;
#pragma unroll
    for (int r = 0; r < A; ++r)
#pragma unroll
      for (int qq = 0; qq < A; ++qq) {
        f32x4 acc = {0.f, 0.f, 0.f, 0.f};
        bool first = true;
#pragma unroll
        for (int k = 0; k < A; ++k) axpy(acc, first, W::BT[qq][k], w[r][k]);
        if constexpr (PL) sp::store4(reinterpret_cast<char*>(V) + (r * A + qq) * plane_bytes, t, c, C >> 4, acc);
        else st4(dst + (r * A + qq) * plane, acc);
      }
  }
}

template <int MT, int R>
__global__ __launch_bounds__(256) void wino_output_kernel(const float* __restrict__ M, int N4, Geom g,
                                                          const float* __restrict__ bias, int relu,
                                                          const float* __restrict__ mask, int ld_mask,
                                                          float* __restrict__ out, int ld_out, int Nreal,
                                                          int accumulate, unsigned int* __restrict__ gate_out,
                                                          int ld_gate, const unsigned int* __restrict__ mask_bits,
                                                          int ld_mask_bits, float* __restrict__ pool_out, int ld_pool,
                                                          long long total, const int* __restrict__ tile_list = nullptr,
                                                          long long Tc = 0) {
  using W = WT<MT, R>;
  constexpr int A = W::A;
  constexpr int MP = MT / 2;
  const int N = N4 * 4;
  const long long plane = (tile_list ? Tc : g.T) * N;
  const int sub = threadIdx.x & 7;
  for (long long i = (long long)blockIdx.x * blockDim.x + threadIdx.x; i < total;
       i += (long long)gridDim.x * blockDim.x) {
    const int n = (int)(i % N4) * 4;
    const long long t = i / N4;
    const long long tg = tile_list ? (long long)tile_list[t] : t;
    const int tx = (int)(tg % g.tw);
    const long long q = tg / g.tw;
    const int ty = (int)(q % g.th);
    const int b = (int)(q / g.th);
    const float* src = M + t * N + n;
    f32x4 rr[MT][A];
#pragma unroll
    for (int s = 0; s < A; ++s) {
      f32x4 m[A];
#pragma unroll
      for (int k = 0; k < A; ++k) m[k] = ld4(src + (k * A + s) * plane);
#pragma unroll
      for (int a = 0; a < MT; ++a) {
        f32x4 acc = {0.f, 0.f, 0.f, 0.f};
        bool first = true;
#pragma unroll
        for (int k = 0; k < A; ++k) axpy(acc, first, W::AT[a][k], m[k]);
        rr[a][s] = acc;
      }
    }
    f32x4 bv = {0.f, 0.f, 0.f, 0.f};
    if (bias) {
#pragma unroll
      for (int e = 0; e < 4; ++e) bv[e] = (n + e < Nreal) ? bias[n + e] : 0.f;
    }
    f32x4 pm[MP][MP];
#pragma unroll
    for (int a = 0; a < MT; ++a) {
      const int oy = MT * ty + a;
      if (oy >= g.OH) continue;
#pragma unroll
      for (int cc = 0; cc < MT; ++cc) {
        const int ox = MT * tx + cc;
        if (ox >= g.OW) continue;
        f32x4 v = {0.f, 0.f, 0.f, 0.f};
        bool first = true;
#pragma unroll
        for (int k = 0; k < A; ++k) axpy(v, first, W::AT[cc][k], rr[a][k]);
        v += bv;
        const long long m = ((long long)b * g.OH + oy) * g.OW + ox;
        if (accumulate) {
          v += ld4(out + m * ld_out + n);
        }
        if (relu) {
#pragma unroll
          for (int e = 0; e < 4; ++e) v[e] = fmaxf(v[e], 0.f);
        }
        if (mask_bits) {
          const unsigned int wbits = mask_bits[m * ld_mask_bits + (n >> 5)] >> (n & 31);
#pragma unroll
          for (int e = 0; e < 4; ++e) v[e] = ((wbits >> e) & 1u) ? v[e] : 0.f;
        }
        if (gate_out) {
          unsigned int nib = 0u;
#pragma unroll
          for (int e = 0; e < 4; ++e) nib |= (n + e < Nreal && v[e] > 0.f) ? (1u << e) : 0u;
          unsigned int word = nib << (4 * sub);
          word |= __shfl_xor(word, 1, 64);
          word |= __shfl_xor(word, 2, 64);
          word |= __shfl_xor(word, 4, 64);
          if (sub == 0) gate_out[m * ld_gate + (n >> 5)] = word;
        }
        if (n + 3 < Nreal) {
          if (mask) {
            const f32x4 mk = ld4(mask + m * ld_mask + n);
#pragma unroll
            for (int e = 0; e < 4; ++e) v[e] = (mk[e] > 0.f) ? v[e] : 0.f;
          }
          st4(out + m * ld_out + n, v);
        } else {
          for (int e = 0; e < 4 && n + e < Nreal; ++e) {
            float xv = v[e];
            if (mask) xv = (mask[m * ld_mask + n + e] > 0.f) ? xv : 0.f;
            out[m * ld_out + n + e] = xv;
          }
        }
        if (pool_out) {
          if ((a & 1) == 0 && (cc & 1) == 0) pm[a >> 1][cc >> 1] = v;
          else {
#pragma unroll
            for (int e = 0; e < 4; ++e) pm[a >> 1][cc >> 1][e] = fmaxf(pm[a >> 1][cc >> 1][e], v[e]);
          }
          if ((a & 1) && (cc & 1)) {
            const long long pm_ = ((long long)b * (g.OH >> 1) + (oy >> 1)) * (g.OW >> 1) + (ox >> 1);
            st4(pool_out + pm_ * ld_pool + n, pm[a >> 1][cc >> 1]);
          }
        }
      }
    }
  }
}

constexpr int ADJ_SEG = 8;

__global__ __launch_bounds__(256) void wino_adjoint_output_kernel(const float* __restrict__ Pm, int C4, int Bn, int th,
                                                                  int tw, int IH, int IW, const float* __restrict__ mask,
                                                                  int ld_mask, const unsigned int* __restrict__ mask_bits,
                                                                  int ld_mask_bits, float* __restrict__ out, int ld_out,
                                                                  int Creal, long long total) {
  using W = WT<4, 3>;
  constexpr int A = 6;
  const int C = C4 * 4;
  const int bh = (IH + 3) / 4, bw = (IW + 3) / 4;
  const int nseg = (bh + ADJ_SEG - 1) / ADJ_SEG;
  const long long plane = (long long)Bn * th * tw * C;
  for (long long i = (long long)blockIdx.x * blockDim.x + threadIdx.x; i < total;
       i += (long long)gridDim.x * blockDim.x) {
    const int c = (int)(i % C4) * 4;
    long long t = i / C4;
    const int bx = (int)(t % bw);
    long long q = t / bw;
    const int sg = (int)(q % nseg);
    const int b = (int)(q / nseg);
    const int by0 = sg * ADJ_SEG, by1 = min(by0 + ADJ_SEG, bh);
    f32x4 carry[2][4];
#pragma unroll
    for (int a = 0; a < 2; ++a)
#pragma unroll
      for (int e = 0; e < 4; ++e) carry[a][e] = f32x4{0.f, 0.f, 0.f, 0.f};
    for (int ty = by0 - 1; ty < by1; ++ty) {
      f32x4 d[A][4];
#pragma unroll
      for (int a = 0; a < A; ++a)
#pragma unroll
        for (int e = 0; e < 4; ++e) d[a][e] = f32x4{0.f, 0.f, 0.f, 0.f};
      if (ty >= 0 && ty < th) {
#pragma unroll
        for (int ux = 0; ux < 2; ++ux) {
          const int tx = bx - ux;
          if (tx < 0 || tx >= tw) continue;
          const float* src = Pm + (((long long)b * th + ty) * tw + tx) * C + c;
#pragma unroll
          for (int s2 = 0; s2 < A; ++s2) {
            f32x4 pcol[A], wcol[A];
#pragma unroll
            for (int r = 0; r < A; ++r) pcol[r] = ld4(src + (r * A + s2) * plane);
#pragma unroll
            for (int a = 0; a < A; ++a) {
              f32x4 v = {0.f, 0.f, 0.f, 0.f};
              bool first = true;
#pragma unroll
              for (int r = 0; r < A; ++r) axpy(v, first, W::BT[r][a], pcol[r]);
              wcol[a] = v;
            }
#pragma unroll
            for (int e = 0; e < 4; ++e) {
              if (ux && e >= 2) continue;
              const float coef = ux ? W::BT[s2][4 + (e & 1)] : W::BT[s2][e];
#pragma unroll
              for (int a = 0; a < A; ++a) {
                bool first = false;
                axpy(d[a][e], first, coef, wcol[a]);
              }
            }
          }
        }
      }
      if (ty >= by0) {
#pragma unroll
        for (int a = 0; a < 4; ++a) {
          const int y = 4 * ty + a;
          if (y >= IH) continue;
#pragma unroll
          for (int e = 0; e < 4; ++e) {
            const int x = 4 * bx + e;
            if (x >= IW) continue;
            f32x4 v = d[a][e];
            if (a < 2) v += carry[a][e];
            const long long m = ((long long)b * IH + y) * IW + x;
            if (mask_bits) {
              const unsigned int wbits = mask_bits[m * ld_mask_bits + (c >> 5)] >> (c & 31);
#pragma unroll
              for (int k = 0; k < 4; ++k) v[k] = ((wbits >> k) & 1u) ? v[k] : 0.f;
            }
            if (c + 3 < Creal) {
              if (mask) {
                const f32x4 mk = ld4(mask + m * ld_mask + c);
#pragma unroll
                for (int k = 0; k < 4; ++k) v[k] = (mk[k] > 0.f) ? v[k] : 0.f;
              }
              st4(out + m * ld_out + c, v);
            } else {
              for (int k = 0; k < 4 && c + k < Creal; ++k) {
                float xv = v[k];
                if (mask) xv = (mask[m * ld_mask + c + k] > 0.f) ? xv : 0.f;
                out[m * ld_out + c + k] = xv;
              }
            }
          }
        }
      }
#pragma unroll
      for (int e = 0; e < 4; ++e) { carry[0][e] = d[4][e]; carry[1][e] = d[5][e]; }
    }
  }
}

template <int MT, int R, bool PL = false>
__global__ __launch_bounds__(256) void wino_dy_kernel(const float* __restrict__ dy, int ld_dy, int N4,
                                                      Geom g, float* __restrict__ Md,
                                                      float* __restrict__ dbias, int Nreal,
                                                      long long total, long long plane_bytes = 0) {
  using W = WT<MT, R>;
  constexpr int A = W::A;
  extern __shared__ float bacc[];
  const int N = N4 * 4;
  const long long plane = g.T * N;
  if (dbias) {
    for (int k = threadIdx.x; k < N; k += blockDim.x) bacc[k] = 0.f;
    __syncthreads();
  }
  for (long long i = (long long)blockIdx.x * blockDim.x + threadIdx.x; i < total;
       i += (long long)gridDim.x * blockDim.x) {
    int n;
    long long t;
    if constexpr (PL) {
      sp::item_to_row_channel(i, N, t, n);
      if (t >= g.T) continue;
    } else {
      n = (int)(i % N4) * 4;
      t = i / N4;
    }
    const int tx = (int)(t % g.tw);
    const long long q = t / g.tw;
    const int ty = (int)(q % g.th);
    const int b = (int)(q / g.th);
    f32x4 d[MT][MT];
    f32x4 sum = {0.f, 0.f, 0.f, 0.f};
#pragma unroll
    for (int a = 0; a < MT; ++a)
#pragma unroll
      for (int c = 0; c < MT; ++c) {
        const int oy = MT * ty + a, ox = MT * tx + c;
        f32x4 v = {0.f, 0.f, 0.f, 0.f};
        if (oy < g.OH && ox < g.OW) v = ld4(dy + (((long long)b * g.OH + oy) * g.OW + ox) * ld_dy + n);
        d[a][c] = v;
        sum += v;
      }
    if (dbias) {
#pragma unroll
      for (int e = 0; e < 4; ++e) atomicAdd(&bacc[n + e], sum[e]);
    }
    f32x4 w[A][MT];
#pragma unroll
    for (int c = 0; c < MT; ++c)
#pragma unroll
      for (int r = 0; r < A; ++r) {
        f32x4 acc = {0.f, 0.f, 0.f, 0.f};
        bool first = true;
#pragma unroll
        for (int a = 0; a < MT; ++a) axpy(acc, first, W::AT[a][r], d[a][c]);
        w[r][c] = acc;
      }
    float* dst = Md + t * N + n;
#pragma unroll
    for (int r = 0; r < A; ++r)
#pragma unroll
      for (int qq = 0; qq < A; ++qq) {
        f32x4 acc = {0.f, 0.f, 0.f, 0.f};
        bool first = true;
#pragma unroll
        for (int c = 0; c < MT; ++c) axpy(acc, first, W::AT[c][qq], w[r][c]);
        if constexpr (PL) sp::store4(reinterpret_cast<char*>(Md) + (r * A + qq) * plane_bytes, t, n, N >> 4, acc);
        else st4(dst + (r * A + qq) * plane, acc);
      }
  }
  if (dbias) {
    __syncthreads();
    for (int k = threadIdx.x; k < Nreal; k += blockDim.x)
      if (bacc[k] != 0.f) atomicAdd(dbias + k, bacc[k]);
  }
}

template <int MT, int R, bool PL = false>
__global__ __launch_bounds__(256) void wino_dy_dual_kernel(const float* __restrict__ dy, int ld_dy, int N4,
                                                           Geom gd, Geom gw, float* __restrict__ Vd,
                                                           float* __restrict__ Md, float* __restrict__ dbias,
// ... 278 lines not shown
    if (d->N % 64 != 0 || d->src[0].C % 64 != 0 || d->N < 128 || d->src[0].C < 128) return false;
  } else if (d->precision != CLX_PREC_F32X3BF16 || d->N % 128 != 0 || d->src[0].C % 128 != 0) {
    return false;
  }
  const int mt = d->algo == CLX_ALGO_WINOGRAD ? 2 : 4;
  const long long eh = d->IH + (d->PH ? d->KH - 1 : 0), ew = d->IW + (d->PW ? d->KW - 1 : 0);
  const long long tiles = (long long)d->B * ((eh + mt - 1) / mt) * ((ew + mt - 1) / mt);
  const int ch = d->N > d->src[0].C ? d->N : d->src[0].C;
  return sp::planes_bytes(tiles, ch) < (1ll << 32);
}
inline long long sp_items(long long rows, int C) { return (rows + 7) / 8 * 8 * (C / 4); }

clx_conv_desc gemm_desc(float* V, int C, const clx_conv_desc* d, const Geom& gin) {
  clx_conv_desc gd = {};
  gd.nsrc = 1;
  gd.src[0].ptr = V; gd.src[0].C = C; gd.src[0].ld = C;
  gd.src[0].D = d->ID; gd.src[0].H = 1; gd.src[0].W = gin.th * gin.tw;
  gd.src[0].fz = gd.src[0].fy = gd.src[0].fx = 1;
  gd.B = d->B; gd.ID = d->ID; gd.IH = 1; gd.IW = gin.th * gin.tw;
  gd.KD = d->KD; gd.KH = gd.KW = 1;
  gd.PD = d->PD;
  return gd;
}

template <int MT, int R>
int wino_fwd_t(const clx_conv_desc* d, hipStream_t st) {
  constexpr int AA = WT<MT, R>::A * WT<MT, R>::A;
  const Geom gin = geom(d, MT, d->ID), gout = geom(d, MT, out_planes(d));
  const clx_src& S = d->src[0];
  const int C = S.C, Np = pad4(d->N);
  const bool spx = wino_sp(d);
  CLX_REQUIRE(!spx || d->wplanes != nullptr, "clx_conv_fwd(winograd): precision f32x3bf16 needs wplanes (the planes of wpack)");
  float* V = d->vcache ? (float*)d->vcache : (float*)d->workspace;
  const int* list = d->tile_list;
  if (list != nullptr) {
    CLX_REQUIRE(d->KD == 1 && d->ID == 1 && d->PH == 0 && d->vcache == nullptr && !d->accumulate && d->tile_count >= 0 &&
                    d->tile_count <= gin.T && gin.T == gout.T,
                "clx_conv_fwd(winograd): tile_list needs a 2-D valid convolution without vcache / accumulate and at most "
                "th * tw * B tiles");
    if (d->tile_count == 0) return CLX_OK;
  }
  const long long Tin = list ? d->tile_count : gin.T, Tout = list ? d->tile_count : gout.T;
  const long long pbV = spx ? sp::planes_bytes(Tin, C) : 0;
  float* M = spx ? (float*)((char*)d->workspace + AA * sp::planes_bytes(gin.T, C)) : (float*)d->workspace + AA * Tin * C;
  if (!(d->vcache && d->vcache_valid)) {
    if (spx) {
      const long long tot_in = sp_items(Tin, C);
      int rc = clx_sp_zero_tail(V, Tin, C, AA, pbV, st);
      if (rc) return rc;
      CLX_LAUNCH_KIND(CLX_PROF_WINO_TRANSFORM, (wino_input_kernel<MT, R, true>), dim3(grid_for(tot_in, 256)), dim3(256), 0, st, S.ptr, S.ld, C / 4,
                      gin, V, tot_in, list, Tin, pbV);
    } else {
      const long long tot_in = Tin * (C / 4);
      CLX_LAUNCH_KIND(CLX_PROF_WINO_TRANSFORM, (wino_input_kernel<MT, R>), dim3(grid_for(tot_in, 256)), dim3(256), 0, st, S.ptr, S.ld, C / 4, gin, V,
                      tot_in, list, Tin, 0ll);
    }
  }
  if (spx) {
    clx_conv_desc ep = {};
    ep.out = M; ep.ld_out = Np;
    const int rc = clx_sp_launch(V, d->wplanes, (int)Tin, d->N, C, Tin, AA, pbV, sp::planes_bytes(Np, C), Tout * Np, &ep, st);
    if (rc) return rc;
  } else {
    clx_conv_desc gd = gemm_desc(V, C, d, gin);
    if (list) {
      gd.B = 1;
      gd.src[0].W = gd.IW = (int)Tin;
    }
    gd.N = d->N; gd.wpack = d->wpack; gd.out = M; gd.ld_out = Np;
    const int rc = clx_igemm_launch(&gd, AA, Tin * C, (long long)Np * d->KD * C, Tout * Np, st);
    if (rc) return rc;
  }
  const long long tot_out = Tout * (Np / 4);
  CLX_REQUIRE((d->gate_out == nullptr && d->mask_bits == nullptr) || Np % 32 == 0,
              "clx_conv_fwd(winograd): gate_out / mask_bits need a channel count that is a multiple of 32");
  CLX_REQUIRE(d->gate_out == nullptr || d->relu, "clx_conv_fwd(winograd): gate_out needs relu");
  if (d->pool_out != nullptr) {
    CLX_REQUIRE(d->KD == 1 && d->ID == 1 && gout.OH % 2 == 0 && gout.OW % 2 == 0,
                "clx_conv_fwd(winograd): pool_out needs a 2-D layer with even output height and width");
    CLX_REQUIRE(d->N % 4 == 0 && d->ld_pool % 4 == 0 && d->ld_pool >= d->N && ((uintptr_t)d->pool_out & 15) == 0 &&
                    d->mask == nullptr && d->mask_bits == nullptr && !d->accumulate,
                "clx_conv_fwd(winograd): pool_out needs N %% 4 == 0, an aligned ld_pool >= N, and no mask / accumulate");
  }
  CLX_LAUNCH_KIND(CLX_PROF_WINO_TRANSFORM, (wino_output_kernel<MT, R>), dim3(grid_for(tot_out, 256)), dim3(256), 0, st, M, Np / 4, gout, d->bias,
                  d->relu, d->mask, d->ld_mask, d->out, d->ld_out, d->N, d->accumulate, d->gate_out, d->ld_gate, d->mask_bits,
                  d->ld_mask_bits, d->pool_out, d->ld_pool, tot_out, list, Tout);
  CLX_CHECK_LAUNCH("clx_conv_fwd(winograd)");
  return CLX_OK;
}

template <int MT, int R>
int wino_wgrad_t(const clx_conv_desc* d, const float* dy, int ld_dy, float* dwpack, float* dbias, hipStream_t st) {
  constexpr int AA = WT<MT, R>::A * WT<MT, R>::A;
  const Geom gin = geom(d, MT, d->ID), gout = geom(d, MT, out_planes(d));
  const clx_src& S = d->src[0];
  const int C = S.C, N = d->N;
  const bool spx = wino_sp(d);
  float* V = d->vcache ? (float*)d->vcache : (float*)d->workspace;
  const long long pbV = spx ? sp::planes_bytes(gin.T, C) : 0, pbM = spx ? sp::planes_bytes(gout.T, N) : 0;
  float* Md = spx ? (float*)((char*)d->workspace + AA * pbV) : (float*)d->workspace + AA * gin.T * C;
  if (!(d->vcache && d->vcache_valid)) {
    if (spx) {
      const long long tot_in = sp_items(gin.T, C);
      int rc = clx_sp_zero_tail(V, gin.T, C, AA, pbV, st);
      if (rc) return rc;
      CLX_LAUNCH_KIND(CLX_PROF_WINO_TRANSFORM, (wino_input_kernel<MT, R, true>), dim3(grid_for(tot_in, 256)), dim3(256), 0, st, S.ptr, S.ld, C / 4,
                      gin, V, tot_in, (const int*)nullptr, 0ll, pbV);
    } else {
      const long long tot_in = gin.T * (C / 4);
      CLX_LAUNCH_KIND(CLX_PROF_WINO_TRANSFORM, (wino_input_kernel<MT, R>), dim3(grid_for(tot_in, 256)), dim3(256), 0, st, S.ptr, S.ld, C / 4, gin, V,
                      tot_in, (const int*)nullptr, 0ll, 0ll);
    }
  }
  if (spx) {
    const int rc = clx_sp_zero_tail(Md, gout.T, N, AA, pbM, st);
    if (rc) return rc;
  }
  if (d->dy_vcache) {
    Geom gd = gout;
    gd.SH = gout.OH; gd.SW = gout.OW; gd.oy = gd.ox = 0;
    gd.ID = gd.SD = out_planes(d); gd.oz = 0;
    gd.IH = gout.OH; gd.IW = gout.OW; gd.P = R - 1;
    gd.OH = gout.OH + R - 1; gd.OW = gout.OW + R - 1;
    gd.th = (gd.OH + MT - 1) / MT; gd.tw = (gd.OW + MT - 1) / MT;
    gd.T = (long long)gd.B * gd.th * gd.tw;
    const long long tot = spx ? sp_items(gd.T, N) : gd.T * (N / 4);
    int blocks = grid_for(tot, 256);
    if (dbias && blocks > 2048) blocks = 2048;
    if (spx) {
      const long long pbD = sp::planes_bytes(gd.T, N);
      const int rc = clx_sp_zero_tail(d->dy_vcache, gd.T, N, AA, pbD, st);
      if (rc) return rc;
      CLX_LAUNCH_KIND(CLX_PROF_WINO_TRANSFORM, (wino_dy_dual_kernel<MT, R, true>), dim3(blocks), dim3(256), (size_t)N * sizeof(float), st, dy, ld_dy,
                      N / 4, gd, gout, (float*)d->dy_vcache, Md, dbias, N, tot, pbD, pbM);
    } else {
      CLX_LAUNCH_KIND(CLX_PROF_WINO_TRANSFORM, (wino_dy_dual_kernel<MT, R>), dim3(blocks), dim3(256), (size_t)N * sizeof(float), st, dy, ld_dy, N / 4,
                      gd, gout, (float*)d->dy_vcache, Md, dbias, N, tot, 0ll, 0ll);
    }
  } else {
    const long long tot_dy = spx ? sp_items(gout.T, N) : gout.T * (N / 4);
    int blocks = grid_for(tot_dy, 256);
    if (blocks > 2048) blocks = 2048;
    if (spx)
      CLX_LAUNCH_KIND(CLX_PROF_WINO_TRANSFORM, (wino_dy_kernel<MT, R, true>), dim3(blocks), dim3(256), (size_t)N * sizeof(float), st, dy, ld_dy, N / 4,
                      gout, Md, dbias, N, tot_dy, pbM);
    else
      CLX_LAUNCH_KIND(CLX_PROF_WINO_TRANSFORM, (wino_dy_kernel<MT, R>), dim3(blocks), dim3(256), (size_t)N * sizeof(float), st, dy, ld_dy, N / 4, gout,
                      Md, dbias, N, tot_dy, 0ll);
  }
  if (spx) {
    CLX_REQUIRE(gin.T == gout.T, "clx_conv_wgrad(winograd): tile counts of input and output differ");
    CLX_REQUIRE(d->det_turns == nullptr, "clx_conv_wgrad: the reproducible mode exists for the float32 precision only");
    const int rc = clx_sp_wgrad_launch(Md, V, gin.T, N, C, AA, pbM, pbV, (long long)N * C, dwpack, C, st);
    if (rc) return rc;
    CLX_CHECK_LAUNCH("clx_conv_wgrad(winograd, split precision)");
    return CLX_OK;
  }
  clx_conv_desc gd = gemm_desc(V, C, d, gin);
  gd.N = N;
  gd.det_turns = d->det_turns;
  const int rc = clx_wgrad_launch(&gd, Md, N, dwpack, nullptr, AA, gin.T * C, gout.T * N,
                                  (long long)d->KD * N * C, st);
  if (rc) return rc;
  CLX_CHECK_LAUNCH("clx_conv_wgrad(winograd)");
  return CLX_OK;
}

}

bool clx_wino_sp(const clx_conv_desc* d) { return wino_sp(d); }

extern "C" size_t clx_conv_workspace_bytes(const clx_conv_desc* d, int pass) {
  if (d == nullptr || !applicable(d)) return 0;
  if (pass == CLX_PASS_WGRAD && d->PH != 0) return 0;
  const int mt = tile_of(d), a = mt + d->KH - 1;
  const Geom gin = geom(d, mt, d->ID), gout = geom(d, mt, out_planes(d));
  if (gout.OH <= 0 || gout.OW <= 0 || out_planes(d) <= 0 || gin.T >= (1ll << 31) || gout.T >= (1ll << 31)) return 0;
  const long long C = d->src[0].C, N = pad4(d->N);
  if (wino_sp(d)) {
    const long long v = sp::planes_bytes(gin.T, (int)C);
    const long long m = pass == CLX_PASS_WGRAD ? sp::planes_bytes(gout.T, (int)N) : gout.T * N * (long long)sizeof(float);
    return (size_t)(a * a * (v + m));
  }
  return (size_t)(a * a * (gin.T * C + gout.T * N)) * sizeof(float);
}

extern "C" size_t clx_conv_vcache_bytes(const clx_conv_desc* d, int which) {
  if (d == nullptr || !applicable(d)) return 0;
  const int mt = tile_of(d), a = mt + d->KH - 1, R = d->KH;
  const Geom gin = geom(d, mt, d->ID), gout = geom(d, mt, out_planes(d));
  const long long C = d->src[0].C, N = pad4(d->N);
  if (which == 0) return wino_sp(d) ? (size_t)(a * a * sp::planes_bytes(gin.T, (int)C)) : (size_t)(a * a * gin.T * C) * sizeof(float);
  const long long th = (gout.OH + R - 1 + mt - 1) / mt, tw = (gout.OW + R - 1 + mt - 1) / mt;
  const long long Td = (long long)gout.B * th * tw;
  return wino_sp(d) ? (size_t)(a * a * sp::planes_bytes(Td, (int)N)) : (size_t)(a * a * Td * N) * sizeof(float);
}

static int wino_adjoint(const clx_conv_desc* d, hipStream_t st) {
  CLX_REQUIRE(d->algo == CLX_ALGO_WINOGRAD4 && d->KH == 3 && d->KW == 3 && d->PH == 2 && d->PW == 2 && d->nsrc == 1 &&
                  ((d->KD == 1 && d->ID == 1 && d->PD == 0) || (d->KD == 3 && d->PD == 2)),
              "clx_conv_fwd(adjoint): a 3x3 (2-D) or 3x3x3 layer in its data-gradient form (padding 2) with "
              "CLX_ALGO_WINOGRAD4 only");
  CLX_REQUIRE(d->bias == nullptr && !d->relu && !d->accumulate && d->gate_out == nullptr,
              "clx_conv_fwd(adjoint): only the ReLU-gate epilogues (mask / mask_bits) exist");
  CLX_REQUIRE(d->N % 4 == 0 && d->src[0].C % 4 == 0, "clx_conv_fwd(adjoint): channel counts must be multiples of 4");
  const int OHf = d->IH, OWf = d->IW;
  const int th = (OHf + 3) / 4, tw = (OWf + 3) / 4;
  const int planes_dy = d->ID, planes_dx = d->ID + 2 * d->PD - (d->KD - 1);
  const long long Tdy = (long long)d->B * planes_dy * th * tw, Tdx = (long long)d->B * planes_dx * th * tw;
  const int Nf = d->src[0].C, Cp = d->N;
  const bool spx = wino_sp(d);
  const size_t need = spx ? (size_t)36 * (sp::planes_bytes(Tdx, Cp) + sp::planes_bytes(Tdy, Nf))
                          : (size_t)36 * (Tdx * Cp + Tdy * Nf) * sizeof(float);
  CLX_REQUIRE(d->workspace != nullptr && d->workspace_bytes >= need && ((uintptr_t)d->workspace & 15) == 0,
              "clx_conv_fwd(adjoint): needs the %zu workspace bytes of the layer's weight gradient (%zu given)", need,
              d->workspace_bytes);
  CLX_REQUIRE(d->mask_bits == nullptr || Cp % 32 == 0, "clx_conv_fwd(adjoint): mask_bits needs whole words per pixel");
  float* P = (float*)d->workspace;
  float* Mdy = P + (size_t)36 * Tdx * Cp;
  if (spx) {
    CLX_REQUIRE(d->wplanes != nullptr, "clx_conv_fwd(adjoint): precision f32x3bf16 needs wplanes");
    const char* Mp = (const char*)d->workspace + 36 * sp::planes_bytes(Tdx, Cp);
    clx_conv_desc ep = {};
    ep.out = P; ep.ld_out = Cp;
    const int rc = clx_sp_launch(Mp, d->wplanes, (int)Tdy, Cp, Nf, Tdy, 36, sp::planes_bytes(Tdy, Nf), sp::planes_bytes(Cp, Nf),
                                 Tdx * Cp, &ep, st);
    if (rc) return rc;
  } else {
  clx_conv_desc gd = {};
  gd.nsrc = 1;
  gd.src[0].ptr = Mdy; gd.src[0].C = Nf; gd.src[0].ld = Nf;
  gd.src[0].D = planes_dy; gd.src[0].H = 1; gd.src[0].W = th * tw;
  gd.src[0].fz = gd.src[0].fy = gd.src[0].fx = 1;
  gd.B = d->B; gd.ID = planes_dy; gd.IH = 1; gd.IW = th * tw;
  gd.KD = d->KD; gd.KH = gd.KW = 1; gd.PD = d->PD;
  gd.N = Cp; gd.wpack = d->wpack; gd.out = P; gd.ld_out = Cp;
  const int rc = clx_igemm_launch(&gd, 36, Tdy * Nf, (long long)Cp * d->KD * Nf, Tdx * Cp, st);
  if (rc) return rc;
  }
  const int IH = OHf + 2, IW = OWf + 2;
  const int nseg = ((IH + 3) / 4 + ADJ_SEG - 1) / ADJ_SEG;
  const long long total = (long long)d->B * planes_dx * nseg * ((IW + 3) / 4) * (Cp / 4);
  CLX_LAUNCH_KIND(CLX_PROF_WINO_TRANSFORM, wino_adjoint_output_kernel, dim3(grid_for(total, 256)), dim3(256), 0, st, P, Cp / 4,
                  d->B * planes_dx, th, tw, IH, IW, d->mask, d->ld_mask, d->mask_bits, d->ld_mask_bits, d->out, d->ld_out, Cp, total);
  CLX_CHECK_LAUNCH("clx_conv_fwd(winograd adjoint)");
  return CLX_OK;
}

int clx_wino_fwd(const clx_conv_desc* d, hipStream_t st) {
  if (d->adjoint) return wino_adjoint(d, st);
  CLX_REQUIRE(applicable(d), "clx_conv_fwd: Winograd does not apply to this geometry");
  const size_t need = clx_conv_workspace_bytes(d, CLX_PASS_FWD);
  CLX_REQUIRE(d->workspace != nullptr && d->workspace_bytes >= need && need > 0,
              "clx_conv_fwd: Winograd needs %zu workspace bytes (%zu given)", need, d->workspace_bytes);
  CLX_REQUIRE(((uintptr_t)d->workspace & 15) == 0 && ((uintptr_t)d->vcache & 15) == 0,
              "clx_conv_fwd: workspace / vcache must be 16-byte aligned");
  if (d->KH == 2) return wino_fwd_t<4, 2>(d, st);
  return tile_of(d) == 4 ? wino_fwd_t<4, 3>(d, st) : wino_fwd_t<2, 3>(d, st);
}

int clx_wino_wgrad(const clx_conv_desc* d, const float* dy, int ld_dy, float* dwpack, float* dbias,
                   hipStream_t st) {
  CLX_REQUIRE(applicable(d) && d->PH == 0, "clx_conv_wgrad: Winograd does not apply to this geometry");
  const size_t need = clx_conv_workspace_bytes(d, CLX_PASS_WGRAD);
  CLX_REQUIRE(d->workspace != nullptr && d->workspace_bytes >= need && need > 0,
              "clx_conv_wgrad: Winograd needs %zu workspace bytes (%zu given)", need, d->workspace_bytes);
  CLX_REQUIRE(((uintptr_t)d->workspace & 15) == 0 && ((uintptr_t)d->vcache & 15) == 0,
              "clx_conv_wgrad: workspace / vcache must be 16-byte aligned");
  CLX_REQUIRE(d->N <= 8192, "clx_conv_wgrad: too many output channels for the Winograd bias accumulator");
  if (d->KH == 2) return wino_wgrad_t<4, 2>(d, dy, ld_dy, dwpack, dbias, st);
  return tile_of(d) == 4 ? wino_wgrad_t<4, 3>(d, dy, ld_dy, dwpack, dbias, st)
                         : wino_wgrad_t<2, 3>(d, dy, ld_dy, dwpack, dbias, st);
}

int clx_wino_pack(const float* w, float* wp, int cout, int cin, int cin_pad, int cout_pad, int dgrad,
                  int tile, int ksize, int kd, hipStream_t st) {
  const bool fused = dgrad == 3;
  if (fused) dgrad = 0;
  const int rows = dgrad ? cin_pad : cout_pad, cols = dgrad ? cout_pad : cin_pad;
  const long long total = (long long)rows * kd * cols;
  const int grid = grid_for(total, 256);
  if (ksize == 2) wino_filter_kernel<4, 2><<<grid, 256, 0, st>>>(w, wp, cout, cin, rows, cols, kd, dgrad, total, fused);
  else if (tile == 4) wino_filter_kernel<4, 3><<<grid, 256, 0, st>>>(w, wp, cout, cin, rows, cols, kd, dgrad, total, fused);
  else wino_filter_kernel<2, 3><<<grid, 256, 0, st>>>(w, wp, cout, cin, rows, cols, kd, dgrad, total, fused);
  return CLX_OK;
}

extern "C" int clx_pack_weights_batch(const clx_pack_job* jobs, int njobs, long long max_total, clx_stream stream) {
  CLX_REQUIRE(jobs != nullptr && njobs > 0 && njobs < 65536 && max_total > 0, "clx_pack_weights_batch: bad arguments");
  CLX_REQUIRE(((uintptr_t)jobs & 7) == 0, "clx_pack_weights_batch: the job table must be 8-byte aligned");
  long long gx = (max_total + 255) / 256;
  if (gx > 512) gx = 512;
  pack_batch_kernel<<<dim3((unsigned)gx, (unsigned)njobs), 256, 0, (hipStream_t)stream>>>(jobs);
  CLX_CHECK_LAUNCH("clx_pack_weights_batch");
  return CLX_OK;
}

extern "C" int clx_unpack_wgrad_wino(const float* du, float* dw, int cout, int cin, int rows,
                                     int cin_pad, int tile, int ksize, int kd, clx_stream stream) {
  CLX_REQUIRE(du && dw, "clx_unpack_wgrad_wino: null pointer");
  CLX_REQUIRE(cout > 0 && cin > 0 && rows >= cout && cin_pad >= cin, "clx_unpack_wgrad_wino: bad extents");
  CLX_REQUIRE((ksize == 3 && (tile == 2 || tile == 4)) || (ksize == 2 && tile == 4),
              "clx_unpack_wgrad_wino: (tile, ksize) must be (2, 3), (4, 3) or (4, 2)");
  CLX_REQUIRE(kd == 1 || (kd == ksize && tile == 4), "clx_unpack_wgrad_wino: kd must be 1 or ksize (F(4x4) only)");
  const long long total = (long long)cout * cin * kd;
  const int grid = grid_for(total, 256);
  hipStream_t st = (hipStream_t)stream;
  if (ksize == 2) wino_unpack_kernel<4, 2><<<grid, 256, 0, st>>>(du, dw, cout, cin, rows, cin_pad, kd, total);
  else if (tile == 4) wino_unpack_kernel<4, 3><<<grid, 256, 0, st>>>(du, dw, cout, cin, rows, cin_pad, kd, total);
  else wino_unpack_kernel<2, 3><<<grid, 256, 0, st>>>(du, dw, cout, cin, rows, cin_pad, kd, total);
  CLX_CHECK_LAUNCH("clx_unpack_wgrad_wino");
  return CLX_OK;
}
```

### cellulus_amd/models/plan.py

```python

import ctypes
import math
import os
from dataclasses import dataclass, field
from typing import List, Tuple

import torch

from .. import _clx
from .._clx import ClxConvDesc, ClxSrc


def pad4(c: int) -> int:
    return (c + 3) // 4 * 4


WINO_MIN_CHANNELS = int(os.environ.get("CLX_WINOGRAD_MIN_CHANNELS", "64"))
WINO_TAPS = {1: 16, 2: 36, 3: 36}
WINO_PACK_FWD = {1: 2, 2: 4, 3: 7}
WINO_PACK_DGRAD = {1: 3, 2: 5}
WINO_TILE = {1: 2, 2: 4, 3: 4}


WINO_MIN_CHANNELS_3D = int(os.environ.get("CLX_WINOGRAD_MIN_CHANNELS_3D", "64"))
# ... 183 lines not shown
        for d in range(3):
            if target[d] <= conv_crop[d] and up_shape[d] != target[d]:
                raise RuntimeError(f"Feature map with shape {up_shape} is too small for cropping to factor")
        up_crop = tuple((s - t) // 2 for s, t in zip(up_shape, target))
        skip, skip_c, skip_shape = left_out[i]
        for d in range(3):
            if skip_shape[d] < target[d]:
                raise RuntimeError("skip connection smaller than the upsampled feature map")
        skip_crop = tuple((s - t) // 2 for s, t in zip(skip_shape, target))
        cout = features_in_last_layer if i == 0 else num_fmaps * fmap_inc_factor ** i
        srcs = [Source(skip, skip_c, crop=skip_crop),
                Source(below, below_c, crop=up_crop, factor=f)]
        layers = add_pass(f"backbone.r_conv.0.{i}", srcs, target, cout, f"r{i}")
        topo.r_info[i] = dict(conv0=layers[0], skip=skip, up=below, level=i)
        below, below_c, below_shape = layers[-1].out, cout, layers[-1].out_shape

    top, top_c, top_shape = below, below_c, below_shape
    if L > 0 and top_c != features_in_last_layer:
        raise AssertionError("internal: top level width mismatch")
    h0 = ConvLayer(name="head.0", sources=[Source(top, top_c)], cout=features_in_last_layer,
                   kernel=k1, in_shape=top_shape, out="h0", relu=True)
    h1 = ConvLayer(name="head.2", sources=[Source("h0", features_in_last_layer)], cout=out_channels,
                   kernel=k1, in_shape=top_shape, out="h1", relu=False)
    if L == 0 and top_c != features_in_last_layer:
        raise ValueError("with no downsampling, num_fmaps must equal features_in_last_layer")
    for layer in (h0, h1):
        topo.convs.append(layer)
        topo.fwd_order.append(layer)
        topo.shapes[layer.out] = (layer.out_shape, layer.cout)
    topo.out_shape = top_shape
    for idx, layer in enumerate(topo.convs):
        layer.param_index = idx
    return topo


def tensor_consumers(topo):
    n = {}
    for layer in topo.convs:
        for src in layer.sources:
            n[src.tensor] = n.get(src.tensor, 0) + 1
    for pool in topo.pools:
        n[pool.src] = n.get(pool.src, 0) + 1
    return n


def find_chain_pairs(topo, algo_fwd, batch):
    produced_by_conv = {layer.out: layer for layer in topo.convs}
    readers = tensor_consumers(topo)
    one = (1, 1, 1)
    plain = lambda s: tuple(s.crop) == (0, 0, 0) and tuple(s.factor) == (1, 1, 1)
    pairs = []
    i = 0
    while i + 1 < len(topo.convs):
        a, b = topo.convs[i], topo.convs[i + 1]
        ok = (tuple(a.kernel) == one and tuple(b.kernel) == one and len(a.sources) == 1 and len(b.sources) == 1
              and plain(a.sources[0]) and plain(b.sources[0]) and b.sources[0].tensor == a.out
              and a.sources[0].tensor in produced_by_conv and a.sources[0].channels == 64 and a.cout == 64
              and a.relu and (b.cout == 64 or b.cout <= 8)
              and readers.get(a.out, 0) == 1 and readers.get(a.sources[0].tensor, 0) == 1
              and not algo_fwd[a.name] and not algo_fwd[b.name]
              and batch * a.in_shape[0] * a.in_shape[1] * a.in_shape[2] < (1 << 31) - 256)
        if ok:
            pairs.append((a, b))
            i += 2
        else:
            i += 1
    return pairs


class UNetPlan:

    def __init__(self, topo: Topology, batch: int, device: torch.device, keep_activations: bool):
        self.topo = topo
        self.B = int(batch)
        self.device = device
        self.keep = keep_activations
        self.precision = precision_code()
        self.fused = fused_wanted(keep_activations)
        self.deterministic = os.environ.get("CLX_DETERMINISTIC", "0") == "1"
        self._wplanes = {}
        self.aplanes = None
        self.xplanes = {}
        self._xplanes_fresh = set()
        self.dyplanes = None
        self.dyplanes2 = None
        self._pointwise_reader = {}
        self.dx_bufs = {}
        self.buf = {}
        self._alloc()

    def _fused_ok(self, cin_pad, cout):
        return bool(self.fused and not self.precision and fused_pays(cin_pad, cout))

    def _alloc(self):
        t = self.topo
        for name, (shape, c) in t.shapes.items():
            n = self.B * shape[0] * shape[1] * shape[2]
            self.buf[name] = _clx.zeros((n, pad4(c)), torch.float32, self.device)
        self.algo = {}
        self.workspace = None
        ws_bytes = 0
        for layer in t.convs:
            a = dict(fwd=0, dgrad=0, wgrad=0)
            if (winograd_enabled() and min(layer.cin_pad, layer.cout) >= wino_min_channels(layer.kernel)
                    and (layer.kernel[0] == 1 or winograd_code() == 2)):
                lib = _clx.load()
                code = winograd_code()
                d = self._desc(layer)
                d.algo = code
                d.N = layer.cout
                nf = int(lib.clx_conv_workspace_bytes(ctypes.byref(d), 0))
                if nf:
                    a["fwd"], ws_bytes = code, max(ws_bytes, nf)
                    if (code == 2 and self._fused_ok(layer.cin_pad, layer.cout) and layer.cout == pad4(layer.cout)
                            and int(lib.clx_conv_fused_applicable(ctypes.byref(d)))):
                        a["fwd"] = 3
                        ws_bytes = max(ws_bytes, int(lib.clx_conv_fused_workspace_bytes(ctypes.byref(d))))
                d.N = pad4(layer.cout)
                nw = int(lib.clx_conv_workspace_bytes(ctypes.byref(d), 1))
                if nw and self.keep:
                    a["wgrad"], ws_bytes = code, max(ws_bytes, nw)
                if self.keep and layer.param_index > 0:
                    dd = self._dgrad_desc(layer, None)
                    dd.algo = code
                    nd_ = int(lib.clx_conv_workspace_bytes(ctypes.byref(dd), 0))
                    if nd_:
                        a["dgrad"], ws_bytes = code, max(ws_bytes, nd_)
            self.algo[layer.name] = a
        self.subpixel = {}
        for info in t.r_info:
            sp = self._subpixel_geometry(info["conv0"])
            if sp is not None:
                self.subpixel[info["conv0"].name] = sp
                n = self.B * sp["zshape"][0] * sp["zshape"][1] * sp["zshape"][2]
                self.buf[sp["zname"]] = _clx.zeros((n, sp["P"] * sp["N"]), torch.float32, self.device)
                sp["wino"] = 0
                sp["fused_z"] = sp["fused_skip"] = False
                if (winograd_enabled() and winograd_code() == 2 and sp["zk"] in ((1, 2, 2), (2, 2, 2))
                        and min(sp["C1p"], sp["P"] * sp["N"]) >= wino_min_channels(sp["zk"])):
                    lib = _clx.load()
                    dz, _ds = self._sp_descs(info["conv0"], sp)
                    dz.algo = 2
                    need = [int(lib.clx_conv_workspace_bytes(ctypes.byref(dz), 0))]
                    if self.keep:
                        need.append(int(lib.clx_conv_workspace_bytes(ctypes.byref(dz), 1)))
                        dl = self._sp_low_dgrad_desc(info["conv0"], sp, None)
                        dl.algo = 2
                        need.append(int(lib.clx_conv_workspace_bytes(ctypes.byref(dl), 0)))
                    if all(need):
                        sp["wino"] = 2
                        ws_bytes = max([ws_bytes] + need)
                        sp["fused_z"] = bool(self._fused_ok(sp["C1p"], sp["P"] * sp["N"])
                                             and int(lib.clx_conv_fused_applicable(ctypes.byref(dz))))
                        if sp["fused_z"]:
                            ws_bytes = max(ws_bytes, int(lib.clx_conv_fused_workspace_bytes(ctypes.byref(dz))))
                sp["wino_skip"] = 0
                conv0 = info["conv0"]
                if (winograd_enabled() and winograd_code() == 2 and tuple(conv0.kernel) in ((1, 3, 3), (3, 3, 3))
                        and sp["C0p"] >= wino_min_channels(conv0.kernel)
                        and sp["N"] >= wino_min_channels(conv0.kernel) // 2):
                    lib = _clx.load()
                    _dz, ds = self._sp_descs(conv0, sp)
                    ds.algo = 2
                    ds.N = conv0.cout
                    need = [int(lib.clx_conv_workspace_bytes(ctypes.byref(ds), 0))]
                    if self.keep:
# ... 806 lines not shown
            if readers.get(src, 0) != 1:
                break
            tail.append(op)
            src = op.out
        return (first, tail) if tail else None

    def first_layer_on_rows(self):
        prefix = self.pointwise_prefix()
        if prefix is None or os.environ.get("CLX_SPARSE_FIRST", "1") == "0":
            return False
        first = prefix[0]
        return (self.topo.in_channels == 1 and tuple(first.kernel) in ((1, 3, 3), (3, 3, 3)) and first.cout % 4 == 0
                and first.in_shape[0] >= first.kernel[0])

    def tiled_layer_behind_prefix(self):
        prefix = self.pointwise_prefix()
        if prefix is None:
            return None
        first, tail = prefix
        ops = self.topo.fwd_order
        k = 1 + len(tail)
        if k >= len(ops) or not isinstance(ops[k], ConvLayer):
            return None
        op = ops[k]
        code = self.algo[op.name]["fwd"]
        if (not code or op.kernel[0] != 1 or op.in_shape[0] != 1 or op.name in self.subpixel or op.name in self.chains
                or op.name in self.chain_second or len(op.sources) != 1):
            return None
        s = op.sources[0]
        if s.tensor != tail[-1].out or tuple(s.crop) != (0, 0, 0) or tuple(s.factor) != (1, 1, 1):
            return None
        return op, WINO_TILE[code]

    def _compact(self, slot, rows, width):
        bufs = self.__dict__.setdefault("_compact_bufs", {})
        b = bufs.get(slot)
        if b is None or b.shape[0] < rows or b.shape[1] != width:
            b = bufs[slot] = _clx.zeros((max(rows, 1), width), torch.float32, self.device)
        return b

    def forward_prefix(self, raw, params, nlayers):
        t = self.topo
        st = _clx.stream_ptr(self.device)
        npix_in = t.in_shape[0] * t.in_shape[1] * t.in_shape[2]
        raw = raw.contiguous()
        _clx.call("clx_planar_to_pixel", _clx.ptr(raw), _clx.ptr(self.buf["raw"]), self.B,
                  t.in_channels, npix_in, pad4(t.in_channels), st)
        for op in t.fwd_order[:1 + nlayers]:
            self._conv_forward(op, params, st)
        return self.buf[t.fwd_order[nlayers].out]

    def _conv_forward(self, op, params, st, tiles=None):
        d = self._desc(op)
        d.N = op.cout
        self._set_wpack(d, self.wpack_fwd[op.name])
        b = params[2 * op.param_index + 1]
        d.bias = b.data_ptr() if b is not None else None
        d.relu = 1 if op.relu else 0
        d.mask = None
        d.ld_mask = 0
        d.out = self.buf[op.out].data_ptr()
        d.ld_out = pad4(op.cout)
        if op.relu and self.keep:
            self._set_gate_out(d, op.out)
        if self.sp_pass[op.name][0] and not self.algo[op.name]["fwd"]:
            xp = self.xplanes.get(op.name) if self.keep and self._bwd_ready and tiles is None else None
            d.aplanes = (xp if xp is not None else self.aplanes).data_ptr()
            if xp is not None:
                d.aplanes_valid = 1 if op.name in self._xplanes_fresh else 0
                self._xplanes_fresh.add(op.name)
                nxt = self._pointwise_reader.get(op.out)
                if nxt is not None and os.environ.get("CLX_SP_EPILOGUE_PLANES", "1") != "0":
                    d.out_planes = self.xplanes[nxt.name].data_ptr()
                    self._xplanes_fresh.add(nxt.name)
        if self.algo[op.name]["fwd"]:
            self._use_workspace(d, self.algo[op.name]["fwd"])
            if self.keep and self._bwd_ready and op.name in self.vcache:
                d.vcache = self.vcache[op.name].data_ptr()
                self._vcache_fresh.add(op.name)
            pool = self.fused_pool.get(op.name)
            if pool is not None:
                d.pool_out = self.buf[pool.out].data_ptr()
                d.ld_pool = pad4(pool.channels)
        if tiles is not None:
            d.tile_list = tiles[0].data_ptr()
            d.tile_count = int(tiles[1])
        _clx.call("clx_conv_fwd", ctypes.byref(d), st)

    def _tiles_forward(self, op, params, sparse, st):
        dense = self.buf[op.out]
        clean = sparse["clean_tile_rows"]
        assert clean.shape[1] == dense.shape[1] and clean.shape[0] * self.B == dense.shape[0]
        _clx.call("clx_broadcast_rows", _clx.ptr(clean), clean.numel(), _clx.ptr(dense), self.B, st)
        pool = self.fused_pool.get(op.name)
        if pool is not None:
            pooled, clean_pooled = self.buf[pool.out], sparse["clean_pool_rows"]
            assert clean_pooled.shape[0] * self.B == pooled.shape[0]
            _clx.call("clx_broadcast_rows", _clx.ptr(clean_pooled), clean_pooled.numel(), _clx.ptr(pooled), self.B, st)
        if int(sparse["ntiles"]) > 0:
            self._conv_forward(op, params, st, tiles=(sparse["tiles"], sparse["ntiles"]))

    def _pointwise_on_rows(self, tail, params, sparse, st):
        n, rows = int(sparse["n"]), sparse["rows"]
        src = self.buf[tail[0].sources[0].tensor]
        width = src.shape[1]
        cur = None
        if n > 0:
            cur = self._compact(0, n, width)
            if sparse.get("noisy") is not None:
                first = self.topo.fwd_order[0]
                b = params[2 * first.param_index + 1]
                _clx.call("clx_grey_rows", _clx.ptr(sparse["noisy"]), self.B, *first.in_shape, first.kernel[0],
                          _clx.ptr(rows), n, _clx.ptr(self.wpack_fwd[first.name]), _clx.ptr(b) if b is not None else None,
                          1 if first.relu else 0, first.cout, _clx.ptr(cur), width, st)
            else:
                _clx.call("clx_gather_rows", _clx.ptr(src), width, _clx.ptr(rows), n, width, _clx.ptr(cur), width, st)
            for k, op in enumerate(tail):
                y = self._compact(1 + k % 2, n, pad4(op.cout))
                d = ClxConvDesc()
                d.nsrc = 1
                src_d = ClxSrc()
                src_d.ptr = cur.data_ptr()
                src_d.C = src_d.ld = cur.shape[1]
                src_d.D, src_d.H, src_d.W = 1, 1, n
                src_d.oz = src_d.oy = src_d.ox = 0
                src_d.fz = src_d.fy = src_d.fx = 1
                d.src[0] = src_d
                d.B = 1
                d.ID, d.IH, d.IW = 1, 1, n
                d.KD = d.KH = d.KW = 1
                d.PD = d.PH = d.PW = 0
                d.N = op.cout
                self._set_wpack(d, self.wpack_fwd[op.name])
                d.precision = self.precision
                if self.precision and self.aplanes is not None:
                    d.aplanes = self.aplanes.data_ptr()
                b = params[2 * op.param_index + 1]
                d.bias = b.data_ptr() if b is not None else None
                d.relu = 1 if op.relu else 0
                d.out = y.data_ptr()
                d.ld_out = y.shape[1]
                _clx.call("clx_conv_fwd", ctypes.byref(d), st)
                cur = y
        dense = self.buf[tail[-1].out]
        clean = sparse["clean_rows"]
        assert clean.shape[1] == dense.shape[1] and clean.shape[0] * self.B == dense.shape[0]
        _clx.call("clx_broadcast_rows", _clx.ptr(clean), clean.numel(), _clx.ptr(dense), self.B, st)
        if n > 0:
            _clx.call("clx_scatter_rows", _clx.ptr(cur), cur.shape[1], _clx.ptr(rows), n, dense.shape[1],
                      _clx.ptr(dense), dense.shape[1], st)

    def forward(self, raw, params, out=None, on_op=None, sparse=None):
        t = self.topo
        st = _clx.stream_ptr(self.device)
        sparse_tail = self.pointwise_prefix()[1] if sparse is not None else None
        self._vcache_fresh = set()
        self._xplanes_fresh = set()
        npix_in = t.in_shape[0] * t.in_shape[1] * t.in_shape[2]
        raw = raw.contiguous()
        rows_only_first = sparse is not None and self.first_layer_on_rows()
        if rows_only_first:
            sparse = dict(sparse, noisy=raw)
        else:
            _clx.call("clx_planar_to_pixel", _clx.ptr(raw), _clx.ptr(self.buf["raw"]), self.B,
                      t.in_channels, npix_in, pad4(t.in_channels), st)
        for op_index, op in enumerate(t.fwd_order):
            if on_op is not None and op_index > 0:
                on_op(op_index - 1)
            if op_index == 0 and rows_only_first:
                continue
            if isinstance(op, ConvLayer) and op.name in self.chain_second:
                continue
            if isinstance(op, ConvLayer) and op.name in self.chains:
                self._chain_forward(*self.chains[op.name], params, st)
            elif isinstance(op, ConvLayer) and op.name in self.subpixel:
                self._sp_forward(op, self.subpixel[op.name], params[2 * op.param_index + 1], st)
            elif isinstance(op, ConvLayer) and sparse_tail and op is sparse_tail[0]:
                self._pointwise_on_rows(sparse_tail, params, sparse, st)
            elif isinstance(op, ConvLayer) and sparse_tail and any(op is q for q in sparse_tail):
                continue
            elif isinstance(op, ConvLayer) and sparse is not None and sparse.get("tiles") is not None \
                    and op is sparse["tile_op"]:
                self._tiles_forward(op, params, sparse, st)
            elif isinstance(op, ConvLayer):
                self._conv_forward(op, params, st)
            elif any(p is op for p in self.fused_pool.values()):
                continue
            else:
                D, H, W = op.in_shape
                _clx.call("clx_maxpool_fwd", _clx.ptr(self.buf[op.src]), _clx.ptr(self.buf[op.out]),
                          self.B, D, H, W, pad4(op.channels), *op.factor, st)
        npix_out = t.out_shape[0] * t.out_shape[1] * t.out_shape[2]
        spatial = t.out_shape[3 - t.nd:]
        if out is None:
            out = torch.empty((self.B, t.out_channels) + tuple(spatial), dtype=torch.float32, device=self.device)
        assert out.is_contiguous() and tuple(out.shape) == (self.B, t.out_channels) + tuple(spatial)
        _clx.call("clx_pixel_to_planar", _clx.ptr(self.buf["h1"]), _clx.ptr(out), self.B,
                  t.out_channels, npix_out, pad4(t.out_channels), st)
        return out

    def backward(self, dout, params, grads, on_layer_done=None, flat_grad=None, dx=None):
        st = _clx.stream_ptr(self.device)
        self.zero_gradients(grads, flat_grad)
        for done, unpack in self.backward_steps(dout, params, grads, dx=dx):
            unpack(st)
            if on_layer_done is not None:
                for i in done:
                    on_layer_done(i)

    def train_pass(self, raw, params, grads, flat_grad, loss_fn, after_loss=None, on_layer_done=None):
        out = self.forward(raw, params)
        dout = loss_fn(out, 0, self.B)
        if after_loss is not None:
            after_loss()
        self.backward(dout, params, grads, on_layer_done=on_layer_done, flat_grad=flat_grad)
        return out

    def zero_gradients(self, grads, flat_grad=None):
        if flat_grad is not None:
            _clx.zero_many(self.dwpack, flat_grad)
        else:
            _clx.zero_many(self.dwpack)
            for g in grads[1::2]:
                if g is not None:
                    g.zero_()

    def first_dgrad(self, layer, dy, w, dx, st):
        assert dx.is_contiguous() and dx.dtype == torch.float32 and dx.shape[0] == self.B
        wv = w.detach()
        if not wv.is_contiguous():
            wv = wv.contiguous()
        OD, OH, OW = layer.out_shape
        if _first_dgrad_kernel_wanted(layer):
            _clx.call("clx_conv_first_dgrad", _clx.ptr(dy), dy.shape[1], _clx.ptr(wv), layer.cout, layer.cin, self.B,
                      OD, OH, OW, layer.kernel[0], _clx.ptr(dx), st)
            return
        if not self.dx_bufs:
            n = self.B * layer.in_shape[0] * layer.in_shape[1] * layer.in_shape[2]
            self.dx_bufs["wpack"] = torch.empty(layer.cin_pad * layer.taps * pad4(layer.cout), dtype=torch.float32,
                                                device=self.device)
# ... 52 lines not shown
            wtaps = wino_taps(wino_w, layer.kernel) if wino_w else layer.taps
            dwp = self.dwpack[off:off + wtaps * pad4(layer.cout) * layer.cin_pad]
            adjoint = layer.name in self.adjoint
            dual = (self.dycache is not None and wino_w and layer.param_index > 0
                    and self.algo[layer.name]["dgrad"] == wino_w and not adjoint)
            if wino_w:
                self._use_workspace(d, wino_w)
                if layer.name in self.vcache and layer.name in self._vcache_fresh:
                    d.vcache = self.vcache[layer.name].data_ptr()
                    d.vcache_valid = 1
                if dual:
                    d.dy_vcache = self.dycache.data_ptr()
            dy_planes = dy_planes_of.pop(layer.out, None)
            dy_ready = dy_planes is not None
            if dy_planes is None and self.dyplanes is not None:
                dy_planes = self.dyplanes
            if self.sp_pass[layer.name][2] and not wino_w:
                d.aplanes = self.xplanes[layer.name].data_ptr()
                d.aplanes_valid = 1 if layer.name in self._xplanes_fresh else 0
                d.dyplanes = dy_planes.data_ptr()
                d.dyplanes_valid = 1 if dy_ready else 0
                if dy_ready:
                    gb = None
                dy_ready = True
            elif dy_ready:
                raise AssertionError("planes of dY were written for a layer whose weight gradient does not read them")
            self._wgrad(d, dy, pad4(layer.cout), dwp, gb, layer.cout, st)
            yield (layer.param_index,), self._unpack_step(layer, dwp, grads[2 * layer.param_index], wino_w)
            if layer.param_index == 0:
                if dx is not None:
                    self.first_dgrad(layer, dy, params[0], dx, st)
                continue
            dd = self._dgrad_desc(layer, dy)
            self._set_wpack(dd, self.wpack_dgrad[layer.name])
            dgrad_sp = self.sp_pass[layer.name][1] and not self.algo[layer.name]["dgrad"]
            if dgrad_sp:
                dd.aplanes = dy_planes.data_ptr()
                dd.aplanes_valid = 1 if dy_ready else 0
            if self.algo[layer.name]["dgrad"]:
                self._use_workspace(dd, self.algo[layer.name]["dgrad"])
                if adjoint:
                    dd.adjoint = 1
                elif dual:
                    dd.vcache = self.dycache.data_ptr()
                    dd.vcache_valid = 1
            if len(layer.sources) == 2:
                info = r_by_conv0[layer.name]
                cat = self.gbuf["cat%d" % info["level"]]
                dd.mask = None
                dd.ld_mask = 0
                dd.out = cat.data_ptr()
                dd.ld_out = layer.cin_pad
                _clx.call("clx_conv_fwd", ctypes.byref(dd), st)
                skip_s, up_s = layer.sources
                ushape, uc = t.shapes[up_s.tensor]
                LD, LH, LW = layer.in_shape
                _clx.call("clx_upsample_bwd", _clx.ptr(cat), layer.cin_pad, pad4(skip_s.channels),
                          LD, LH, LW, *up_s.crop, _clx.ptr(self.buf[up_s.tensor]),
                          _clx.ptr(self.gbuf[up_s.tensor]), self.B, ushape[0], ushape[1], ushape[2],
                          pad4(uc), *up_s.factor, st)
                pending_skip[skip_s.tensor] = (cat, layer.cin_pad, layer)
            else:
                s = layer.sources[0]
                if s.tensor in pool_by_out:
                    pool = pool_by_out[s.tensor]
                    dd.mask = None
                    dd.ld_mask = 0
                    dd.out = self.gbuf[pool.out].data_ptr()
                    dd.ld_out = pad4(pool.channels)
                    _clx.call("clx_conv_fwd", ctypes.byref(dd), st)
                    cat, ld_cat, rl = pending_skip.pop(pool.src)
                    skip_s = rl.sources[0]
                    D, H, W = pool.in_shape
                    SD, SH, SW = rl.in_shape
                    _clx.call("clx_maxpool_bwd", _clx.ptr(self.buf[pool.src]), _clx.ptr(self.buf[pool.out]),
                              _clx.ptr(self.gbuf[pool.out]), _clx.ptr(cat), ld_cat, SD, SH, SW,
                              *skip_s.crop, _clx.ptr(self.gbuf[pool.src]), self.B, D, H, W,
                              pad4(pool.channels), *pool.factor, st)
                else:
                    prev = by_out[s.tensor]
                    self._set_mask(dd, prev.out, relu=prev.relu)
                    dd.out = self.gbuf[prev.out].data_ptr()
                    dd.ld_out = pad4(prev.cout)
                    if (dgrad_sp and prev.name in self.xplanes and self.sp_pass[prev.name][2]
                            and os.environ.get("CLX_SP_EPILOGUE_PLANES", "1") != "0"):
                        other = self.dyplanes2 if dy_planes is self.dyplanes else self.dyplanes
                        dd.out_planes = other.data_ptr()
                        gbp = grads[2 * prev.param_index + 1]
                        dd.out_colsum = gbp.data_ptr() if gbp is not None else None
                        dy_planes_of[prev.out] = other
                    _clx.call("clx_conv_fwd", ctypes.byref(dd), st)
        assert not pending_skip


def _first_dgrad_kernel_wanted(layer):
    return layer.cin <= 4 and os.environ.get("CLX_FIRST_DGRAD", "1") != "0"


def forward_flops(topo, batch):
    total = 0
    for layer in topo.convs:
        m = batch * layer.out_shape[0] * layer.out_shape[1] * layer.out_shape[2]
        total += 2 * m * layer.cout * layer.cin * layer.taps
    return total


class _Rows:

    def __init__(self, parts, attr):
        self._parts, self._attr = parts, attr

    def __getitem__(self, name):
        return torch.cat([getattr(p, self._attr)[name] for p in self._parts], dim=0)

    def __contains__(self, name):
        return name in getattr(self._parts[0], self._attr)

    def __bool__(self):
        return bool(getattr(self._parts[0], self._attr))

    def get(self, name, default=None):
        return self[name] if name in self else default

    def keys(self):
        return getattr(self._parts[0], self._attr).keys()


def dual_stream_wanted(topo, batch, keep_activations):
    if not keep_activations or batch < 2 or batch % 2 or os.environ.get("CLX_STREAMS", "2") == "1":
        return False
    if os.environ.get("CLX_DETERMINISTIC", "0") == "1":
        return False
    return forward_flops(topo, batch // 2) >= float(os.environ.get("CLX_STREAMS_MIN_GFLOP", "100")) * 1e9


class DualPlan:

    def __init__(self, topo, batch, device, keep_activations):
        assert batch % 2 == 0 and keep_activations
        self.topo, self.B, self.device, self.keep = topo, int(batch), device, True
        self.parts = [UNetPlan(topo, batch // 2, device, True) for _ in range(2)]
        self.streams = [torch.cuda.Stream(device=device) for _ in range(2)]
        self._events = [[], [], []]
        self._shared = False
        self.buf = _Rows(self.parts, "buf")

    def __getattr__(self, name):
        if name in ("parts", "streams"):
            raise AttributeError(name)
        if name == "gbuf":
            return _Rows(self.parts, "gbuf")
        return getattr(self.parts[0], name)

    def pack_weights(self, params, version, need_dgrad):
        a, b = self.parts
        a.pack_weights(params, version, need_dgrad)
        if need_dgrad and not self._shared:
            b._alloc_backward()
            b.share_from(a)
            self._shared = True
        b._packed_version = a._packed_version

    def _fork(self):
        main = torch.cuda.current_stream(self.device)
        for s in self.streams:
            s.wait_stream(main)
        return main

    def _join(self, main):
        for s in self.streams:
            main.wait_stream(s)

    def forward(self, raw, params, out=None):
        t = self.topo
        assert self._shared, "pack_weights(need_dgrad=True) must run before forward"
# ... 81 lines not shown
```

### include/clx.h

```cpp
#ifndef CLX_H
#define CLX_H

#include <stddef.h>
#include <stdint.h>

#ifdef __cplusplus
extern "C" {
#endif

typedef void* clx_stream;

enum clx_status {
  CLX_OK = 0,
  CLX_ERR_ARG = -1,
  CLX_ERR_LAUNCH = -2,
  CLX_ERR_WORKSPACE = -3
};

const char* clx_last_error(void);
int clx_abi_version(void);
int clx_device_count(void);

enum clx_profile_kind {
  CLX_PROF_IGEMM_WIDE = 0,
  CLX_PROF_IGEMM_NARROW = 1,
  CLX_PROF_WGRAD = 2,
  CLX_PROF_GEMM_SP = 3,
  CLX_PROF_WGRAD_SP = 4,
  CLX_PROF_SPLIT_PLANES = 5,
  CLX_PROF_CHAIN64 = 6,
  CLX_PROF_MS_PREPARE = 7,
  CLX_PROF_MS_ASSIGN = 8,
  CLX_PROF_CC = 9,
  CLX_PROF_GROW_SHRINK = 10,
  CLX_PROF_MINMAX = 11,
  CLX_PROF_HISTOGRAM = 12,
  CLX_PROF_NOISE_STATS = 13,
  CLX_PROF_WINO_FUSED = 14,
  CLX_PROF_WINO_TRANSFORM = 15,
  CLX_PROF_GEMM_SP2 = 16
};
int clx_profile_enable(int on);
int clx_profile_read(int kind, double* launches, double* total_ms, double* total_flops);
int clx_profile_clock(double* shader_ticks, double* wall_ticks_100mhz, int reset);


typedef struct clx_src {
  const float* ptr;
  int C;
  int ld;
  int D, H, W;
  int oz, oy, ox;
  int fz, fy, fx;
} clx_src;

typedef struct clx_conv_desc {
  int nsrc;
  clx_src src[2];
  int B;
  int ID, IH, IW;
  int KD, KH, KW;
  int PD, PH, PW;
  int N;
  const float* wpack;
  const float* bias;
  int relu;
  const float* mask;
  int ld_mask;
  float* out;
  int ld_out;
  int accumulate;
  int algo;
  void* workspace;
  size_t workspace_bytes;
  void* vcache;
  int vcache_valid;
  int c_real;
  void* dy_vcache;
  unsigned int* gate_out;
  int ld_gate;
  const unsigned int* mask_bits;
  int ld_mask_bits;
  int* det_turns;
  int adjoint;
  float* pool_out;
  int ld_pool;
  const int* tile_list;
  int tile_count;
  int precision;
  const void* wplanes;
  void* aplanes;
  int aplanes_valid;
  void* dyplanes;
  int dyplanes_valid;
  void* out_planes;
  float* out_colsum;
} clx_conv_desc;

enum clx_conv_precision { CLX_PREC_F32 = 0, CLX_PREC_F32X3BF16 = 1, CLX_PREC_F32X3BF16_G64 = 2 };

enum clx_conv_algo {
  CLX_ALGO_DIRECT = 0,
  CLX_ALGO_WINOGRAD = 1,
  CLX_ALGO_WINOGRAD4 = 2,
  CLX_ALGO_WINOGRAD4_FUSED = 3
};
int clx_conv_fused_applicable(const clx_conv_desc* d);
size_t clx_conv_fused_workspace_bytes(const clx_conv_desc* d);
enum clx_conv_pass { CLX_PASS_FWD = 0, CLX_PASS_WGRAD = 1 };
size_t clx_conv_workspace_bytes(const clx_conv_desc* d, int pass);
size_t clx_conv_vcache_bytes(const clx_conv_desc* d, int which);

size_t clx_planes_bytes(long long rows, int K);
int clx_split_planes(const float* x, long long ld, long long rows, int K, void* planes, clx_stream stream);
int clx_join_planes(const void* planes, long long rows, int K, float* x, long long ld, clx_stream stream);
int clx_gemm_planes(const void* a_planes, const void* b_planes, int M, int N, int K, const float* bias, int relu,
                    float* out, int ld_out, clx_stream stream);
int clx_wgrad_planes(const void* dy_planes, const void* x_planes, long long rows, int N, int C, float* dw, int ld_dw,
                     clx_stream stream);

int clx_conv_sp_covers(const clx_conv_desc* d, int pass);

int clx_conv_fwd(const clx_conv_desc* d, clx_stream stream);

size_t clx_conv_wgrad_turns_bytes(const clx_conv_desc* d);
size_t clx_colsum_scratch_bytes(int N);
int clx_colsum_ordered(const float* x, int ld, long long M, int N, float* out, void* scratch, clx_stream stream);

int clx_chain64_fwd(const float* x, int ld_x, long long M, const float* w1, const float* b1, float* y1,
                    int ld_y1, unsigned int* gate1, int ld_gate1, const float* w2, const float* b2, int N2,
                    int relu2, float* y2, int ld_y2, unsigned int* gate2, int ld_gate2, clx_stream stream);
int clx_chain64_bwd(const float* dp2, int ld_dp2, int N2, const float* y1, int ld_y1, const float* x,
                    int ld_x, int gate_x, long long M, const float* w2t, const float* w1t, float* dp0,
                    int ld_dp0, float* dw2, float* db2, float* dw1, float* db1, clx_stream stream);

int clx_conv_wgrad(const clx_conv_desc* d, const float* dy, int ld_dy,
                   float* dwpack, float* dbias, clx_stream stream);

enum clx_pack_mode {
  CLX_PACK_FWD = 0,
  CLX_PACK_DGRAD = 1,
  CLX_PACK_WINO_FWD = 2,
  CLX_PACK_WINO_DGRAD = 3,
  CLX_PACK_WINO4_FWD = 4,
  CLX_PACK_WINO4_DGRAD = 5,
  CLX_PACK_WINO4_ADJOINT = 6,
  CLX_PACK_WINO4_FUSED = 7
};
int clx_pack_weights(const float* w, float* wp, int cout, int cin, int taps,
                     int cin_pad, int cout_pad, int mode, clx_stream stream);
typedef struct clx_pack_job {
  const float* w;
  float* wp;
  int cout, cin, taps, cin_pad, cout_pad, mode;
} clx_pack_job;
int clx_pack_weights_batch(const clx_pack_job* jobs, int njobs, long long max_total, clx_stream stream);
int clx_unpack_wgrad(const float* dwpack, float* dw, int cout, int cin, int taps,
                     int rows, int cin_pad, clx_stream stream);
int clx_unpack_wgrad_wino(const float* du, float* dw, int cout, int cin, int rows,
                          int cin_pad, int tile, int ksize, int kd, clx_stream stream);

int clx_planar_to_pixel(const float* planar, float* pixel, int B, int C,
                        long long n, int ld, clx_stream stream);
int clx_pixel_to_planar(const float* pixel, float* planar, int B, int C,
                        long long n, int ld, clx_stream stream);

int clx_depth_to_space(const float* lo, int ld_lo, float* hi, int ld_hi, int B, int D, int H,
                       int W, int N, int fz, int fy, int fx, clx_stream stream);
int clx_space_to_depth(const float* hi, int ld_hi, float* lo, int ld_lo, int B, int D, int H,
                       int W, int N, int fz, int fy, int fx, clx_stream stream);

int clx_subpixel_split_weights(const float* w, float* w_skip, float* weff, int cout, int cin,
                               int C0, int N, int kd, int kh, int kw, int fz, int fy, int fx,
                               clx_stream stream);
int clx_subpixel_fold_grads(const float* g_skip, const float* g_eff, float* gw, int cout, int cin,
                            int C0, int N, int kd, int kh, int kw, int fz, int fy, int fx,
                            clx_stream stream);

int clx_maxpool_fwd(const float* x, float* y, int B, int D, int H, int W, int C,
                    int fz, int fy, int fx, clx_stream stream);
int clx_maxpool_bwd(const float* x, const float* y, const float* dy_pool,
                    const float* dskip, int ld_skip, int SD, int SH, int SW,
                    int cz, int cy, int cx, float* dx, int B, int D, int H,
                    int W, int C, int fz, int fy, int fx, clx_stream stream);
int clx_upsample_bwd(const float* dcat, int ld_cat, int coff, int LD, int LH,
                     int LW, int oz, int oy, int ox, const float* y, float* dy,
                     int B, int D, int H, int W, int C, int fz, int fy, int fx,
                     clx_stream stream);

int clx_gather_add_fwd(const float* offsets, const long long* coords, float* sel,
                       int B, int P, int ND, int Z, int Y, int X, int* oob_count,
                       clx_stream stream);
int clx_gather_add_bwd(const float* dsel, const long long* coords, float* doffsets,
                       int B, int P, int ND, int Z, int Y, int X, int* oob_count,
                       clx_stream stream);
int clx_oce_loss_fwd_bwd(const float* a, const float* r, float* da, double* sums,
                         long long npairs, int ND, float temperature,
                         float reg_weight, float grad_scale, clx_stream stream);
int clx_oce_pairs_fused(const float* offsets, const long long* anchor,
                        const long long* reference, float* doffsets, double* sums,
                        int B, int P, int ND, int Z, int Y, int X,
                        float temperature, float reg_weight, clx_stream stream);
size_t clx_oce_pairs_det_scratch_bytes(int B, int ND, long long npix);
int clx_oce_pairs_fused_det(const float* offsets, const long long* anchor, const long long* reference,
// ... 152 lines not shown
```

Before: 311.5.

## Write split-precision planes from producer conv epilogues and skip unused f32 outputs

Producer kernels (Winograd output transform, the adjoint data-gradient transform, and the single-channel first-layer conv) now also write the 3xbf16 split planes for the next pointwise consumer directly in their epilogues. This removes a separate split pass that re-reads the activation. The adjoint path also accumulates the bias gradient via shared-memory column sums. When only the planes are consumed, the f32 output store is skipped. In exchange the epilogues do more stores, need extra tail-zeroing launches, and the grey kernel uses a new 8-pixel variant.

```diff
diff --git a/cellulus_amd/_clx.py b/cellulus_amd/_clx.py
--- a/cellulus_amd/_clx.py
+++ b/cellulus_amd/_clx.py
@@ -86,6 +86,9 @@
         ("dyplanes_valid", c_int),
         ("out_planes", c_void_p),
         ("out_colsum", c_void_p),
+        ("next_planes", c_void_p),
+        ("next_colsum", c_void_p),
+        ("skip_out", c_int),
     ]
 
 
@@ -112,6 +115,7 @@
     "clx_conv_workspace_bytes": (c_size_t, [POINTER(ClxConvDesc), _I]),
     "clx_conv_vcache_bytes": (c_size_t, [POINTER(ClxConvDesc), _I]),
     "clx_conv_sp_covers": (_I, [POINTER(ClxConvDesc), _I]),
+    "clx_conv_next_planes_ok": (_I, [POINTER(ClxConvDesc)]),
     "clx_planes_bytes": (c_size_t, [_LL, _I]),
     "clx_split_planes": (_I, [_P, _LL, _LL, _I, _P, _P]),
     "clx_join_planes": (_I, [_P, _LL, _I, _P, _LL, _P]),
diff --git a/cellulus_amd/csrc/clx_common.h b/cellulus_amd/csrc/clx_common.h
--- a/cellulus_amd/csrc/clx_common.h
+++ b/cellulus_amd/csrc/clx_common.h
@@ -55,6 +55,9 @@
 
 bool clx_smallc_applicable(const clx_conv_desc* d);
 int clx_smallc_fwd(const clx_conv_desc* d, hipStream_t st);
+bool clx_smallc_grey_rule(const clx_conv_desc* d);
+bool clx_smallc_grey(const clx_conv_desc* d);
+bool clx_wino_next_planes_rule(const clx_conv_desc* d);
 int clx_smallc_wgrad(const clx_conv_desc* d, const float* dy, int ld_dy, float* dwpack,
                      float* dbias, hipStream_t st);
 
diff --git a/cellulus_amd/csrc/conv_igemm.hip b/cellulus_amd/csrc/conv_igemm.hip
--- a/cellulus_amd/csrc/conv_igemm.hip
+++ b/cellulus_amd/csrc/conv_igemm.hip
@@ -506,6 +506,13 @@
   p.accumulate = d->accumulate;
   p.bs_in = p.bs_w = p.bs_out = 0;
   p.flush_every = 0;
+}
+
+extern "C" int clx_conv_next_planes_ok(const clx_conv_desc* d) {
+  if (d == nullptr || d->N <= 0 || d->N % 32 != 0) return 0;
+  if (d->adjoint || d->algo == CLX_ALGO_WINOGRAD || d->algo == CLX_ALGO_WINOGRAD4) return clx_wino_next_planes_rule(d) ? 1 : 0;
+  if (d->algo != CLX_ALGO_DIRECT || d->tile_list != nullptr) return 0;
+  return clx_smallc_grey_rule(d) && d->KD == 1 ? 1 : 0;
 }
 
 extern "C" int clx_conv_fwd(const clx_conv_desc* d, clx_stream stream) {
@@ -530,6 +537,22 @@
                   (d->algo == CLX_ALGO_DIRECT && d->aplanes != nullptr && clx_sp_applicable(d)),
               "clx_conv_fwd: out_planes / out_colsum / aplanes_valid need the split-precision 1x1 product "
               "(clx_conv_sp_covers, wplanes and aplanes)");
+  if (d->next_planes != nullptr) {
+    const bool grey_ptrs = d->algo != CLX_ALGO_DIRECT || d->adjoint ||
+                           (d->mask == nullptr && d->mask_bits == nullptr && d->gate_out == nullptr && clx_smallc_grey(d));
+    CLX_REQUIRE(clx_conv_next_planes_ok(d) && grey_ptrs,
+                "clx_conv_fwd: next_planes is written by the 2-D Winograd forms (no tile_list), the adjoint data gradient "
+                "and the one-channel first-layer kernel only, N %% 32 == 0 (clx_conv_next_planes_ok)");
+    CLX_REQUIRE(((uintptr_t)d->next_planes & 15) == 0, "clx_conv_fwd: next_planes must be 16-byte aligned");
+  }
+  CLX_REQUIRE(d->next_colsum == nullptr || (d->next_planes != nullptr && d->adjoint),
+              "clx_conv_fwd: next_colsum needs next_planes on the adjoint data gradient");
+  if (d->skip_out) {
+    const bool planes = (d->next_planes != nullptr && d->adjoint) || d->out_planes != nullptr;
+    CLX_REQUIRE(planes && d->gate_out == nullptr && d->pool_out == nullptr,
+                "clx_conv_fwd: skip_out needs the planes of the result from the same call (next_planes on the adjoint data "
+                "gradient, out_planes on the split 1x1 product) and excludes gate_out / pool_out");
+  }
   if (d->algo == CLX_ALGO_WINOGRAD4_FUSED) return clx_wino_fused_fwd(d, (hipStream_t)stream);
   if (d->algo != CLX_ALGO_DIRECT) return clx_wino_fwd(d, (hipStream_t)stream);
   CLX_REQUIRE(d->pool_out == nullptr && d->tile_list == nullptr && !d->adjoint,
diff --git a/cellulus_amd/csrc/conv_smallc.hip b/cellulus_amd/csrc/conv_smallc.hip
--- a/cellulus_amd/csrc/conv_smallc.hip
+++ b/cellulus_amd/csrc/conv_smallc.hip
@@ -1,4 +1,5 @@
 #include "clx_common.h"
+#include "sp_planes.h"
 
 namespace {
 
@@ -13,6 +14,7 @@
   const float* bias;
   float* out;
   int ld_out, relu;
+  char* next_planes;
   const float* dy;
   int ld_dy;
   float* dwp;
@@ -226,6 +228,7 @@
   long long base;
 };
 
+template <int PXN = 4>
 __device__ __forceinline__ Run decode_run(const SmallP& p, uint32_t item) {
   const uint32_t q1 = fdiv(item, p.dRX);
   const int rx = (int)(item - q1 * p.RX);
@@ -235,23 +238,25 @@
   const int oz = (int)(q2 - q3 * p.OD);
   const int b = (int)q3;
   Run r;
-  r.ox0 = rx * 4;
+  r.ox0 = rx * PXN;
   r.m0 = ((b * p.OD + oz) * p.OH + oy) * p.OW + r.ox0;
   r.base = (((long long)b * p.D + oz + p.oz) * p.H + oy + p.oy) * p.W + r.ox0 + p.ox;
   return r;
 }
 
-template <int KD>
+template <int KD, int PXN = 4>
 struct GreyLane {
-  static constexpr int R = KD * 3, NP = R * 6, TAPS = R * 3;
+  static constexpr int PW = PXN + 2;
+  static constexpr int R = KD * 3, NP = R * PW, TAPS = R * 3, CQ = 64 / PXN;
+  static_assert(NP <= 64, "one patch value per lane");
   int px, cq, col;
   long long poff;
   __device__ __forceinline__ GreyLane(const SmallP& p) {
     const int lane = threadIdx.x & 63;
-    px = lane >> 4; cq = lane & 15;
+    px = lane / CQ; cq = lane % CQ;
     const int l = lane < NP ? lane : 0;
-    const int r = l / 6;
-    col = l - r * 6;
+    const int r = l / PW;
+    col = l - r * PW;
     const int tz = r / 3, ty = r - tz * 3;
     poff = ((long long)tz * p.H + ty) * p.W;
   }
@@ -260,16 +265,16 @@
     return p.x[(r.base + poff + c) * p.ld_x];
   }
   __device__ __forceinline__ float tap(float pv, int row, int tx) const {
-    return __shfl(pv, row * 6 + tx + px, 64);
+    return __shfl(pv, row * PW + tx + px, 64);
   }
 };
 
-template <int KD>
+template <int KD, int PXN = 4>
 __global__ __launch_bounds__(256) void conv_grey_fwd_kernel(const SmallP p) {
-  using L = GreyLane<KD>;
+  using L = GreyLane<KD, PXN>;
   const L ln(p);
   const int wave = __builtin_amdgcn_readfirstlane(threadIdx.x >> 6);
-  const int n = blockIdx.y * 64 + ln.cq * 4;
+  const int n = blockIdx.y * (L::CQ * 4) + ln.cq * 4;
   const bool live_n = n < p.N;
   f32x4 w[L::TAPS];
 #pragma unroll
@@ -284,7 +289,7 @@
   float pv[3];
 #pragma unroll
   for (int s = 0; s < 2; ++s) {
-    r[s] = decode_run(p, item + s * stride < last ? item + s * stride : last);
+    r[s] = decode_run<PXN>(p, item + s * stride < last ? item + s * stride : last);
     pv[s] = ln.load_patch(p, r[s]);
   }
   while (true) {
@@ -293,7 +298,7 @@
       if (item > last) return;
       const int s2 = (s + 2) % 3;
       const uint32_t nxt = item + 2 * stride;
-      r[s2] = decode_run(p, nxt < last ? nxt : last);
+      r[s2] = decode_run<PXN>(p, nxt < last ? nxt : last);
       pv[s2] = ln.load_patch(p, r[s2]);
       f32x4 acc = bv;
 #pragma unroll
@@ -304,8 +309,10 @@
 #pragma unroll
         for (int e = 0; e < 4; ++e) acc[e] = fmaxf(acc[e], 0.f);
       }
-      if (live_n && r[s].ox0 + ln.px < p.OW)
+      if (live_n && r[s].ox0 + ln.px < p.OW) {
         *reinterpret_cast<f32x4*>(p.out + (size_t)(r[s].m0 + ln.px) * p.ld_out + n) = acc;
+        if (p.next_planes) sp::store4(p.next_planes, r[s].m0 + ln.px, n, p.N >> 4, acc);
+      }
       item += stride;
     }
   }
@@ -429,11 +436,11 @@
          d->PH == 0 && d->PW == 0 && d->N % 4 == 0 && ld_act % 4 == 0;
 }
 
-dim3 grey_grid(SmallP& p) {
-  p.RX = cdiv(p.OW, 4);
+dim3 grey_grid(SmallP& p, int pxn = 4) {
+  p.RX = cdiv(p.OW, pxn);
   p.items = p.B * p.OD * p.OH * p.RX;
   p.dRX = make_fastdiv(p.RX);
-  const int ny = cdiv(p.N, 64);
+  const int ny = cdiv(p.N, 256 / pxn);
   int nx = 768 / ny;
   if (nx < 1) nx = 1;
   if (nx > cdiv(p.items, 4)) nx = cdiv(p.items, 4);
@@ -473,11 +480,24 @@
   return taps > 1 && taps <= MAX_TAPS && d->N >= 4;
 }
 
+bool clx_smallc_grey_rule(const clx_conv_desc* d) { return clx_smallc_applicable(d) && grey_applicable(d, d->ld_out); }
+
+bool clx_smallc_grey(const clx_conv_desc* d) {
+  return clx_smallc_grey_rule(d) && ((uintptr_t)d->out & 15) == 0 && (!d->bias || ((uintptr_t)d->bias & 15) == 0);
+}
+
 int clx_smallc_fwd(const clx_conv_desc* d, hipStream_t st) {
   SmallP p{};
   fill(d, p);
   p.wpack = d->wpack; p.bias = d->bias; p.out = d->out; p.ld_out = d->ld_out; p.relu = d->relu;
-  if (grey_applicable(d, d->ld_out) && ((uintptr_t)d->out & 15) == 0 && (!d->bias || ((uintptr_t)d->bias & 15) == 0)) {
+  if (clx_smallc_grey(d)) {
+    if (d->next_planes) {
+      const int rc = clx_sp_zero_tail(d->next_planes, p.M, p.N, 1, 0, st);
+      if (rc) return rc;
+      p.next_planes = (char*)d->next_planes;
+      conv_grey_fwd_kernel<1, 8><<<grey_grid(p, 8), 256, 0, st>>>(p);
+      return CLX_OK;
+    }
     const dim3 grid = grey_grid(p);
     if (d->KD == 1) conv_grey_fwd_kernel<1><<<grid, 256, 0, st>>>(p);
     else conv_grey_fwd_kernel<3><<<grid, 256, 0, st>>>(p);
diff --git a/cellulus_amd/csrc/gemm_sp.hip b/cellulus_amd/csrc/gemm_sp.hip
--- a/cellulus_amd/csrc/gemm_sp.hip
+++ b/cellulus_amd/csrc/gemm_sp.hip
@@ -137,6 +137,7 @@
   int nbm, nbn;
   char* out_planes;
   float* colsum; int colsum_n;
+  int skip_out;
   unsigned int stride_a, stride_b;
   int total_steps, steps_per_slice, nslices;
 };
@@ -217,7 +218,7 @@
     }
 #pragma unroll
     for (int j = 0; j < PH; ++j)
-      if (live[j]) *reinterpret_cast<f32x4*>(out_base + (size_t)mrow[j] * p.ld_out) = val[j];
+      if (live[j] && !p.skip_out) *reinterpret_cast<f32x4*>(out_base + (size_t)mrow[j] * p.ld_out) = val[j];
     if (p.out_planes) {
 #pragma unroll
       for (int j = 0; j < PH; ++j)
@@ -1088,6 +1089,7 @@
   CLX_REQUIRE(p.zeros != nullptr, "clx_gemm_planes: cannot resolve the device zero buffer");
   p.out_planes = batch == 1 ? (char*)ep->out_planes : nullptr;
   p.colsum = batch == 1 ? ep->out_colsum : nullptr; p.colsum_n = N;
+  p.skip_out = p.out_planes != nullptr && ep->skip_out ? 1 : 0;
   CLX_REQUIRE(p.out_planes == nullptr || ep->ld_out == N, "clx_gemm_planes: out_planes needs a dense output (ld_out == N)");
   p.nbm = cdiv(M, SP_BM); p.nbn = cdiv(N, SP_BN);
   const char* const tile_env = getenv("CLX_SP_TILE");
diff --git a/cellulus_amd/csrc/wino.hip b/cellulus_amd/csrc/wino.hip
--- a/cellulus_amd/csrc/wino.hip
+++ b/cellulus_amd/csrc/wino.hip
@@ -90,7 +90,7 @@
   }
 }
 
-template <int MT, int R>
+template <int MT, int R, bool PL = false>
 __global__ __launch_bounds__(256) void wino_output_kernel(const float* __restrict__ M, int N4, Geom g,
                                                           const float* __restrict__ bias, int relu,
                                                           const float* __restrict__ mask, int ld_mask,
@@ -99,7 +99,7 @@
                                                           int ld_gate, const unsigned int* __restrict__ mask_bits,
                                                           int ld_mask_bits, float* __restrict__ pool_out, int ld_pool,
                                                           long long total, const int* __restrict__ tile_list = nullptr,
-                                                          long long Tc = 0) {
+                                                          long long Tc = 0, char* __restrict__ next_planes = nullptr) {
   using W = WT<MT, R>;
   constexpr int A = W::A;
   constexpr int MP = MT / 2;
@@ -108,8 +108,15 @@
   const int sub = threadIdx.x & 7;
   for (long long i = (long long)blockIdx.x * blockDim.x + threadIdx.x; i < total;
        i += (long long)gridDim.x * blockDim.x) {
-    const int n = (int)(i % N4) * 4;
-    const long long t = i / N4;
+    int n;
+    long long t;
+    if constexpr (PL) {
+      sp::item_to_row_channel(i, N, t, n);
+      if (t >= g.T) continue;
+    } else {
+      n = (int)(i % N4) * 4;
+      t = i / N4;
+    }
     const long long tg = tile_list ? (long long)tile_list[t] : t;
     const int tx = (int)(tg % g.tw);
     const long long q = tg / g.tw;
@@ -180,6 +187,7 @@
             for (int e = 0; e < 4; ++e) v[e] = (mk[e] > 0.f) ? v[e] : 0.f;
           }
           st4(out + m * ld_out + n, v);
+          if constexpr (PL) sp::store4(next_planes, m, n, N >> 4, v);
         } else {
           for (int e = 0; e < 4 && n + e < Nreal; ++e) {
             float xv = v[e];
@@ -209,17 +217,32 @@
                                                                   int tw, int IH, int IW, const float* __restrict__ mask,
                                                                   int ld_mask, const unsigned int* __restrict__ mask_bits,
                                                                   int ld_mask_bits, float* __restrict__ out, int ld_out,
-                                                                  int Creal, long long total) {
+                                                                  int Creal, long long total, long long cols,
+                                                                  char* __restrict__ next_planes, float* __restrict__ colsum,
+                                                                  int skip_out) {
   using W = WT<4, 3>;
   constexpr int A = 6;
+  extern __shared__ float cacc[];
   const int C = C4 * 4;
   const int bh = (IH + 3) / 4, bw = (IW + 3) / 4;
   const int nseg = (bh + ADJ_SEG - 1) / ADJ_SEG;
   const long long plane = (long long)Bn * th * tw * C;
+  if (colsum) {
+    for (int k = threadIdx.x; k < C; k += blockDim.x) cacc[k] = 0.f;
+    __syncthreads();
+  }
   for (long long i = (long long)blockIdx.x * blockDim.x + threadIdx.x; i < total;
        i += (long long)gridDim.x * blockDim.x) {
-    const int c = (int)(i % C4) * 4;
-    long long t = i / C4;
+    int c;
+    long long t;
+    if (next_planes) {
+      sp::item_to_row_channel(i, C, t, c);
+      if (t >= cols) continue;
+    } else {
+      c = (int)(i % C4) * 4;
+      t = i / C4;
+    }
+    f32x4 csum = {0.f, 0.f, 0.f, 0.f};
     const int bx = (int)(t % bw);
     long long q = t / bw;
     const int sg = (int)(q % nseg);
@@ -291,8 +314,12 @@
 #pragma unroll
                 for (int k = 0; k < 4; ++k) v[k] = (mk[k] > 0.f) ? v[k] : 0.f;
               }
-              st4(out + m * ld_out + c, v);
-            } else {
+              if (!skip_out) st4(out + m * ld_out + c, v);
+              if (next_planes) {
+                sp::store4(next_planes, m, c, C >> 4, v);
+                csum += v;
+              }
+            } else if (!skip_out) {
               for (int k = 0; k < 4 && c + k < Creal; ++k) {
                 float xv = v[k];
                 if (mask) xv = (mask[m * ld_mask + c + k] > 0.f) ? xv : 0.f;
@@ -305,6 +332,15 @@
 #pragma unroll
       for (int e = 0; e < 4; ++e) { carry[0][e] = d[4][e]; carry[1][e] = d[5][e]; }
     }
+    if (colsum) {
+#pragma unroll
+      for (int e = 0; e < 4; ++e) atomicAdd(&cacc[c + e], csum[e]);
+    }
+  }
+  if (colsum) {
+    __syncthreads();
+    for (int k = threadIdx.x; k < Creal; k += blockDim.x)
+      if (cacc[k] != 0.f) atomicAdd(colsum + k, cacc[k]);
   }
 }
 
@@ -749,9 +785,19 @@
                     d->mask == nullptr && d->mask_bits == nullptr && !d->accumulate,
                 "clx_conv_fwd(winograd): pool_out needs N %% 4 == 0, an aligned ld_pool >= N, and no mask / accumulate");
   }
+  if (d->next_planes != nullptr) {
+    const int rc = clx_sp_zero_tail(d->next_planes, (long long)gout.B * gout.OH * gout.OW, d->N, 1, 0, st);
+    if (rc) return rc;
+    const long long tot_pl = sp_items(Tout, Np);
+    CLX_LAUNCH_KIND(CLX_PROF_WINO_TRANSFORM, (wino_output_kernel<MT, R, true>), dim3(grid_for(tot_pl, 256)), dim3(256), 0, st, M, Np / 4, gout,
+                    d->bias, d->relu, d->mask, d->ld_mask, d->out, d->ld_out, d->N, d->accumulate, d->gate_out, d->ld_gate, d->mask_bits,
+                    d->ld_mask_bits, d->pool_out, d->ld_pool, tot_pl, (const int*)nullptr, 0ll, (char*)d->next_planes);
+    CLX_CHECK_LAUNCH("clx_conv_fwd(winograd)");
+    return CLX_OK;
+  }
   CLX_LAUNCH_KIND(CLX_PROF_WINO_TRANSFORM, (wino_output_kernel<MT, R>), dim3(grid_for(tot_out, 256)), dim3(256), 0, st, M, Np / 4, gout, d->bias,
                   d->relu, d->mask, d->ld_mask, d->out, d->ld_out, d->N, d->accumulate, d->gate_out, d->ld_gate, d->mask_bits,
-                  d->ld_mask_bits, d->pool_out, d->ld_pool, tot_out, list, Tout);
+                  d->ld_mask_bits, d->pool_out, d->ld_pool, tot_out, list, Tout, (char*)nullptr);
   CLX_CHECK_LAUNCH("clx_conv_fwd(winograd)");
   return CLX_OK;
 }
@@ -836,6 +882,15 @@
 }
 
 bool clx_wino_sp(const clx_conv_desc* d) { return wino_sp(d); }
+
+bool clx_wino_next_planes_rule(const clx_conv_desc* d) {
+  if (d->N <= 0 || d->N % 32 != 0) return false;
+  if (d->adjoint)
+    return d->algo == CLX_ALGO_WINOGRAD4 && d->KH == 3 && d->KW == 3 && d->PH == 2 && d->PW == 2 && d->nsrc == 1 && d->KD == 1 &&
+           d->ID == 1 && d->PD == 0 && d->src[0].C % 4 == 0 && d->N <= 8192;
+  if (d->algo != CLX_ALGO_WINOGRAD && d->algo != CLX_ALGO_WINOGRAD4) return false;
+  return applicable(d) && d->KD == 1 && d->tile_list == nullptr;
+}
 
 extern "C" size_t clx_conv_workspace_bytes(const clx_conv_desc* d, int pass) {
   if (d == nullptr || !applicable(d)) return 0;
@@ -907,9 +962,18 @@
   }
   const int IH = OHf + 2, IW = OWf + 2;
   const int nseg = ((IH + 3) / 4 + ADJ_SEG - 1) / ADJ_SEG;
-  const long long total = (long long)d->B * planes_dx * nseg * ((IW + 3) / 4) * (Cp / 4);
-  CLX_LAUNCH_KIND(CLX_PROF_WINO_TRANSFORM, wino_adjoint_output_kernel, dim3(grid_for(total, 256)), dim3(256), 0, st, P, Cp / 4,
-                  d->B * planes_dx, th, tw, IH, IW, d->mask, d->ld_mask, d->mask_bits, d->ld_mask_bits, d->out, d->ld_out, Cp, total);
+  const long long cols = (long long)d->B * planes_dx * nseg * ((IW + 3) / 4);
+  const long long total = d->next_planes != nullptr ? sp_items(cols, Cp) : cols * (Cp / 4);
+  int blocks = grid_for(total, 256);
+  if (d->next_planes != nullptr) {
+    const int rc = clx_sp_zero_tail(d->next_planes, (long long)d->B * planes_dx * IH * IW, Cp, 1, 0, st);
+    if (rc) return rc;
+  }
+  if (d->next_colsum != nullptr && blocks > 2048) blocks = 2048;
+  CLX_LAUNCH_KIND(CLX_PROF_WINO_TRANSFORM, wino_adjoint_output_kernel, dim3(blocks), dim3(256),
+                  d->next_colsum != nullptr ? (size_t)Cp * sizeof(float) : 0, st, P, Cp / 4,
+                  d->B * planes_dx, th, tw, IH, IW, d->mask, d->ld_mask, d->mask_bits, d->ld_mask_bits, d->out, d->ld_out, Cp, total, cols,
+                  (char*)d->next_planes, d->next_colsum, d->next_planes != nullptr && d->skip_out ? 1 : 0);
   CLX_CHECK_LAUNCH("clx_conv_fwd(winograd adjoint)");
   return CLX_OK;
 }
diff --git a/cellulus_amd/models/plan.py b/cellulus_amd/models/plan.py
--- a/cellulus_amd/models/plan.py
+++ b/cellulus_amd/models/plan.py
@@ -289,6 +289,7 @@
         self.aplanes = None
         self.xplanes = {}
         self._xplanes_fresh = set()
+        self.producer_handovers = []
         self.dyplanes = None
         self.dyplanes2 = None
         self._pointwise_reader = {}
@@ -1261,6 +1262,13 @@
             if pool is not None:
                 d.pool_out = self.buf[pool.out].data_ptr()
                 d.ld_pool = pad4(pool.channels)
+        if self.keep and self._bwd_ready and tiles is None and _producer_planes_wanted():
+            nxt = self._pointwise_reader.get(op.out)
+            if (nxt is not None and not d.out_planes and (d.algo or not d.gate_out)
+                    and _clx.load().clx_conv_next_planes_ok(ctypes.byref(d))):
+                d.next_planes = self.xplanes[nxt.name].data_ptr()
+                self._xplanes_fresh.add(nxt.name)
+                self.producer_handovers.append(op.out)
         if tiles is not None:
             d.tile_list = tiles[0].data_ptr()
             d.tile_count = int(tiles[1])
@@ -1335,6 +1343,7 @@
         sparse_tail = self.pointwise_prefix()[1] if sparse is not None else None
         self._vcache_fresh = set()
         self._xplanes_fresh = set()
+        self.producer_handovers = []
         npix_in = t.in_shape[0] * t.in_shape[1] * t.in_shape[2]
         raw = raw.contiguous()
         rows_only_first = sparse is not None and self.first_layer_on_rows()
@@ -1553,6 +1562,8 @@
                     self._set_mask(dd, prev.out, relu=prev.relu)
                     dd.out = self.gbuf[prev.out].data_ptr()
                     dd.ld_out = pad4(prev.cout)
+                    prev_reads_planes = (prev.param_index > 0 and self.sp_pass[prev.name][1]
+                                         and not self.algo[prev.name]["dgrad"])
                     if (dgrad_sp and prev.name in self.xplanes and self.sp_pass[prev.name][2]
                             and os.environ.get("CLX_SP_EPILOGUE_PLANES", "1") != "0"):
                         other = self.dyplanes2 if dy_planes is self.dyplanes else self.dyplanes
@@ -1560,8 +1571,25 @@
                         gbp = grads[2 * prev.param_index + 1]
                         dd.out_colsum = gbp.data_ptr() if gbp is not None else None
                         dy_planes_of[prev.out] = other
+                        if prev_reads_planes and _producer_planes_wanted():
+                            dd.skip_out = 1
+                    elif (adjoint and prev.name in self.xplanes and self.sp_pass[prev.name][2]
+                            and not self.algo[prev.name]["wgrad"] and _producer_planes_wanted()
+                            and _clx.load().clx_conv_next_planes_ok(ctypes.byref(dd))):
+                        other = self.dyplanes2 if dy_planes is self.dyplanes else self.dyplanes
+                        dd.next_planes = other.data_ptr()
+                        gbp = grads[2 * prev.param_index + 1]
+                        dd.next_colsum = gbp.data_ptr() if gbp is not None else None
+                        dy_planes_of[prev.out] = other
+                        self.producer_handovers.append("d(%s)" % prev.out)
+                        if prev_reads_planes:
+                            dd.skip_out = 1
                     _clx.call("clx_conv_fwd", ctypes.byref(dd), st)
         assert not pending_skip
+
+
+def _producer_planes_wanted():
+    return os.environ.get("CLX_SP_PRODUCER_PLANES", "1") != "0"
 
 
 def _first_dgrad_kernel_wanted(layer):
diff --git a/include/clx.h b/include/clx.h
--- a/include/clx.h
+++ b/include/clx.h
@@ -95,6 +95,9 @@
   int dyplanes_valid;
   void* out_planes;
   float* out_colsum;
+  void* next_planes;
+  float* next_colsum;
+  int skip_out;
 } clx_conv_desc;
 
 enum clx_conv_precision { CLX_PREC_F32 = 0, CLX_PREC_F32X3BF16 = 1, CLX_PREC_F32X3BF16_G64 = 2 };
@@ -120,6 +123,7 @@
                      clx_stream stream);
 
 int clx_conv_sp_covers(const clx_conv_desc* d, int pass);
+int clx_conv_next_planes_ok(const clx_conv_desc* d);
 
 int clx_conv_fwd(const clx_conv_desc* d, clx_stream stream);
 
```

After: 310.2. No clear change (-0.4%).
